# mtlazaro/cg_mrslam

Hardware: AMD Instinct MI355X
Metric: GN iterations/sec on 10k-vertex SE2 graph (final chi2 reported) (higher is better)
Workload: dtype f64; 1 GPU; C2: synthetic 10000-vertex/40000-edge SE2 pose graph per GPU, one step = GraphSLAM::optimize(10) incl. host ordering+symbolic analysis (analysis cache off); graphs=1, parallelism=1 robot sub-graph per GPU x1

## Files before the change

### cg_mrslam_amd/_lib.py

```python
from __future__ import annotations

import ctypes as C
import math
import os
import subprocess

import numpy as np

_HERE = os.path.dirname(os.path.abspath(__file__))
_LIB = None

CGMR_E_CHOLESKY_BASE = -100
CGMR_E_TIMEOUT = -5


class CgmrError(RuntimeError):
    def __init__(self, code, msg):
        super().__init__(f"cgmr error {code}: {msg}")
        self.code = code


def library_path() -> str:
    return os.environ.get("CGMR_LIB") or os.path.join(_HERE, "libcgmr.so")

# ... 746 lines not shown
        return (z, cz, d2) + st

    def observation_covariance(self, poses, fixed, ef, et, meas, info, pair_a, pair_b, obs_kind=None, hyp_meas=None, hyp_info=None,
                               vertex_kind=None, edge_kind=None, kind=None, delta=1.0):
        a, b = self._pair_arrays(pair_a, pair_b)
        n = len(a)
        ok = None if obs_kind is None else np.ascontiguousarray(obs_kind, dtype=np.uint8).reshape(-1)
        if ok is not None and ok.shape != (n,):
            raise ValueError(f"observation kinds: {ok.shape[0]} given for {n} pairs")
        hm = hi = d2 = None
        if hyp_meas is not None:
            hm = np.ascontiguousarray(hyp_meas, dtype=np.float64).reshape(n, 3)
            d2 = np.zeros(n)
        if hyp_info is not None:
            if hm is None:
                raise ValueError("hyp_info needs hyp_meas")
            hi = np.ascontiguousarray(hyp_info, dtype=np.float64).reshape(n, 6)
        z, cz = np.zeros((n, 3)), np.zeros((n, 3, 3))
        st = self._joint_call("cgmr_observation_covariance", poses, fixed, ef, et, meas, info,
                              (C.c_int(n), _ptr(a), _ptr(b), _ptr(ok), _ptr(z), _ptr(cz), _ptr(hm), _ptr(hi), _ptr(d2)), kind, delta,
                              vertex_kind, edge_kind, typed=True)
        return (z, cz, d2) + st

    @staticmethod
    def _adj_bool(words, n):
        if n == 0:
            return np.zeros((0, 0), dtype=bool)
        bits = (words[:, :, None] >> np.arange(64, dtype=np.uint64)) & np.uint64(1)
        return bits.reshape(n, -1)[:, :n].astype(bool)

    @staticmethod
    def _adj_words(adj):
        adj = np.asarray(adj)
        if adj.dtype == np.uint64:
            return np.ascontiguousarray(adj.reshape(adj.shape[0], -1)), adj.shape[0]
        n = adj.shape[0]
        if adj.shape != (n, n):
            raise ValueError(f"adjacency: a square matrix, not {adj.shape}")
        W = (n + 63) // 64
        bits = np.zeros((n, 64 * W), dtype=np.uint64)
        bits[:, :n] = adj.astype(bool)
        words = (bits.reshape(n, W, 64) << np.arange(64, dtype=np.uint64)).sum(axis=2, dtype=np.uint64)
        return np.ascontiguousarray(words), n

    def closure_consistency(self, poses, fixed, ef, et, meas, info, cl_a, cl_b, cl_meas, cl_info, gamma, kind=None, delta=1.0):
        a, b = self._pair_arrays(cl_a, cl_b)
        n = len(a)
        cm = np.ascontiguousarray(cl_meas, dtype=np.float64).reshape(n, 3)
        ci = np.ascontiguousarray(cl_info, dtype=np.float64).reshape(n, 6)
        W = (n + 63) // 64
        d2, words = np.zeros((n, n)), np.zeros((n, W), dtype=np.uint64)
        clique, size, seed = np.full(n, -1, dtype=np.int32), np.zeros(1, dtype=np.int32), np.full(1, -1, dtype=np.int32)
        st = self._joint_call("cgmr_closure_consistency", poses, fixed, ef, et, meas, info,
                              (C.c_int(n), _ptr(a), _ptr(b), _ptr(cm), _ptr(ci), C.c_double(float(gamma)), _ptr(d2), _ptr(words),
                               _ptr(clique), _ptr(size), _ptr(seed)), kind, delta)
        return (d2, self._adj_bool(words, n), clique[:int(size[0])].copy(), int(seed[0])) + st

    def max_clique_greedy(self, adj):
        words, n = self._adj_words(adj)
        clique, size, seed = np.full(n, -1, dtype=np.int32), np.zeros(1, dtype=np.int32), np.full(1, -1, dtype=np.int32)
        self._check(self.lib.cgmr_max_clique_greedy(self.h, C.c_int(n), _ptr(words), _ptr(clique), _ptr(size), _ptr(seed)))
        return clique[:int(size[0])].copy(), int(seed[0])

    def closure_consistency_exact(self, poses, fixed, ef, et, meas, info, cl_a, cl_b, cl_meas, cl_info, gamma,
                                  node_limit=EXACT_DEFAULT_NODE_LIMIT, kind=None, delta=1.0):
        a, b = self._pair_arrays(cl_a, cl_b)
        n = len(a)
        cm = np.ascontiguousarray(cl_meas, dtype=np.float64).reshape(n, 3)
        ci = np.ascontiguousarray(cl_info, dtype=np.float64).reshape(n, 6)
        W = (n + 63) // 64
        d2, words = np.zeros((n, n)), np.zeros((n, W), dtype=np.uint64)
        clique, size, proven = np.full(n, -1, dtype=np.int32), np.zeros(1, dtype=np.int32), np.zeros(1, dtype=np.int32)
        st = self._joint_call("cgmr_closure_consistency_exact", poses, fixed, ef, et, meas, info,
                              (C.c_int(n), _ptr(a), _ptr(b), _ptr(cm), _ptr(ci), C.c_double(float(gamma)), _ptr(d2), _ptr(words),
                               C.c_int64(int(node_limit)), _ptr(clique), _ptr(size), _ptr(proven)), kind, delta)
        return (d2, self._adj_bool(words, n), clique[:int(size[0])].copy(), bool(proven[0])) + st

    def max_clique_exact(self, adj, node_limit=EXACT_DEFAULT_NODE_LIMIT):
        words, n = self._adj_words(adj)
        clique, size, proven = np.full(n, -1, dtype=np.int32), np.zeros(1, dtype=np.int32), np.zeros(1, dtype=np.int32)
        nodes = np.zeros(1, dtype=np.int64)
        self._check(self.lib.cgmr_max_clique_exact(self.h, C.c_int(n), _ptr(words), C.c_int64(int(node_limit)), _ptr(clique),
                                                   _ptr(size), _ptr(proven), _ptr(nodes)))
        return clique[:int(size[0])].copy(), bool(proven[0]), int(nodes[0])

    @staticmethod
    def _inter_arrays(cl_a, peer_pose, peer_cov, cl_meas, cl_info):
        a = np.ascontiguousarray(cl_a, dtype=np.int32).reshape(-1)
        n = len(a)
        pp = np.ascontiguousarray(peer_pose, dtype=np.float64).reshape(n, 3)
        pc = None
        if peer_cov is not None:
            pc = np.ascontiguousarray(peer_cov, dtype=np.float64)
            if pc.shape != (3 * n, 3 * n):
                raise ValueError(f"peer_cov: [{3 * n}, {3 * n}] for {n} candidates, not {pc.shape}")
        cm = np.ascontiguousarray(cl_meas, dtype=np.float64).reshape(n, 3)
        ci = np.ascontiguousarray(cl_info, dtype=np.float64).reshape(n, 6)
        return a, pp, pc, cm, ci

    def closure_consistency_inter(self, poses, fixed, ef, et, meas, info, cl_a, peer_pose, cl_meas, cl_info, gamma, peer_cov=None,
                                  kind=None, delta=1.0):
        a, pp, pc, cm, ci = self._inter_arrays(cl_a, peer_pose, peer_cov, cl_meas, cl_info)
        n = len(a)
        W = (n + 63) // 64
        d2, words = np.zeros((n, n)), np.zeros((n, W), dtype=np.uint64)
        clique, size, seed = np.full(n, -1, dtype=np.int32), np.zeros(1, dtype=np.int32), np.full(1, -1, dtype=np.int32)
        st = self._joint_call("cgmr_closure_consistency_inter", poses, fixed, ef, et, meas, info,
                              (C.c_int(n), _ptr(a), _ptr(pp), _ptr(pc), _ptr(cm), _ptr(ci), C.c_double(float(gamma)), _ptr(d2),
                               _ptr(words), _ptr(clique), _ptr(size), _ptr(seed)), kind, delta)
        return (d2, self._adj_bool(words, n), clique[:int(size[0])].copy(), int(seed[0])) + st

    def closure_consistency_inter_exact(self, poses, fixed, ef, et, meas, info, cl_a, peer_pose, cl_meas, cl_info, gamma,
                                        peer_cov=None, node_limit=EXACT_DEFAULT_NODE_LIMIT, kind=None, delta=1.0):
        a, pp, pc, cm, ci = self._inter_arrays(cl_a, peer_pose, peer_cov, cl_meas, cl_info)
        n = len(a)
        W = (n + 63) // 64
        d2, words = np.zeros((n, n)), np.zeros((n, W), dtype=np.uint64)
        clique, size, proven = np.full(n, -1, dtype=np.int32), np.zeros(1, dtype=np.int32), np.zeros(1, dtype=np.int32)
        st = self._joint_call("cgmr_closure_consistency_inter_exact", poses, fixed, ef, et, meas, info,
                              (C.c_int(n), _ptr(a), _ptr(pp), _ptr(pc), _ptr(cm), _ptr(ci), C.c_double(float(gamma)), _ptr(d2),
                               _ptr(words), C.c_int64(int(node_limit)), _ptr(clique), _ptr(size), _ptr(proven)), kind, delta)
        return (d2, self._adj_bool(words, n), clique[:int(size[0])].copy(), bool(proven[0])) + st

    def set_symbolic_cache(self, on: bool):
        self._check(self.lib.cgmr_set_symbolic_cache(self.h, C.c_int(1 if on else 0)))

    def host_threads_info(self):
        out = np.zeros(5, dtype=np.int32)
        self._check(self.lib.cgmr_host_threads_info(_ptr(out)))
        return {"threads": int(out[0]), "pinned": bool(out[1]), "home_cpu": int(out[2]), "cpus_allowed": int(out[3]),
                "moves": int(out[4])}

    def symbolic_cache_stats(self):
        out = np.zeros(3, dtype=np.int64)
        self._check(self.lib.cgmr_symbolic_cache_stats3(self.h, _ptr(out)))
        return {"hits": int(out[0]), "misses": int(out[1]), "extended": int(out[2])}

    def gn_timeouts(self) -> int:
        self.lib.cgmr_gn_timeouts.restype = C.c_int64
        return int(self.lib.cgmr_gn_timeouts(self.h))

    def switches(self):
        return {r["name"]: r["value"] for r in _switch_rows(self.lib, self.h)}

    def gn_last_timing(self):
        out = np.zeros(5)
        self._check(self.lib.cgmr_gn_last_timing(self.h, _ptr(out)))
        return dict(zip(["order", "structure", "upload", "device", "total"], out.tolist()))

    def set_profiling(self, on: bool):
        self._check(self.lib.cgmr_set_profiling(self.h, C.c_int(1 if on else 0)))

    def gn_kernel_times(self):
        sec = np.zeros(12)
        n = np.zeros(12, dtype=np.int64)
        self._check(self.lib.cgmr_gn_kernel_times_ex(self.h, _ptr(sec), _ptr(n)))
        names = ["linearize", "assemble", "chi2", "front_factor", "front_update", "top_block", "solve_bwd", "update", "front_level"]
        return {k: (float(s), int(c)) for k, s, c in zip(names, sec, n)}

    def pcm_kernel_times(self):
        sec = np.zeros(12)
        n = np.zeros(12, dtype=np.int64)
        self._check(self.lib.cgmr_gn_kernel_times_ex(self.h, _ptr(sec), _ptr(n)))
        return {k: (float(sec[i]), int(n[i])) for i, k in zip((9, 10, 11), ("gram", "consistency", "bits_clique"))}


def _switch_rows(lib, h):
    need = lib.cgmr_switches(h, None, C.c_int(0))
    if need <= 0:
        raise CgmrError(need, "cgmr_switches failed")
    buf = C.create_string_buffer(need)
    lib.cgmr_switches(h, buf, C.c_int(need))
    rows = []
    for line in buf.value.decode().splitlines():
        name, scope, value, effect = line.split("\t")
        rows.append(dict(name=name, scope=scope, value=int(value) if value.lstrip("-").isdigit() else value, effect=effect))
    return rows


def switch_table():
    return _switch_rows(load_library(), None)


_SYM_KEYS = ["free_poses", "offdiag_blocks", "fronts", "levels", "L_doubles", "U_doubles", "max_border",
             "factor_flops", "order_us", "structure_us", "max_children", "max_children_small_border", "panel_doubles",
             "launch_levels", "top_block_fronts", "top_block_cols"]


def gn_symbolic_info_grown(nV0, nE0, nV_steps, nE_steps, ef, et):
    lib = load_library()
    ef = np.ascontiguousarray(ef, dtype=np.int32)
    et = np.ascontiguousarray(et, dtype=np.int32)
    nv = np.ascontiguousarray(nV_steps, dtype=np.int32)
    ne = np.ascontiguousarray(nE_steps, dtype=np.int32)
    out = np.zeros(16, dtype=np.int64)
    nV = int(nv[-1]) if len(nv) else nV0
    perm = np.zeros(nV, dtype=np.int32)
    next_ = C.c_int32(0)
    rc = lib.cgmr_gn_symbolic_info_grown(C.c_int(nV0), C.c_int(nE0), C.c_int(len(nv)), _ptr(nv), _ptr(ne), _ptr(ef), _ptr(et),
                                         _ptr(out), _ptr(perm), C.byref(next_))
    if rc != 0:
        raise CgmrError(rc, "cgmr_gn_symbolic_info_grown rejected the graph")
    return dict(zip(_SYM_KEYS, out.tolist())), perm, int(next_.value)


def gn_front_table(nV, fixed, ef, et):
    lib = load_library()
    fixed = np.ascontiguousarray(fixed, dtype=np.uint8)
    ef = np.ascontiguousarray(ef, dtype=np.int32)
    et = np.ascontiguousarray(et, dtype=np.int32)
    cap = max(64, int(nV))
    out = np.zeros(6 * cap, dtype=np.int32)
    n = lib.cgmr_debug_fronts(C.c_int(nV), _ptr(fixed), C.c_int(len(ef)), _ptr(ef), _ptr(et), C.c_int(cap), _ptr(out))
    if n < 0 or n > cap:
        raise CgmrError(n, "cgmr_debug_fronts rejected the graph")
    return out[:6 * n].reshape(n, 6)


def gn_symbolic_info(nV, fixed, ef, et, want_perm=False):
    lib = load_library()
    fixed = np.ascontiguousarray(fixed, dtype=np.uint8)
    ef = np.ascontiguousarray(ef, dtype=np.int32)
    et = np.ascontiguousarray(et, dtype=np.int32)
    out = np.zeros(16, dtype=np.int64)
    perm = np.zeros(nV, dtype=np.int32) if want_perm else None
    rc = lib.cgmr_gn_symbolic_info(C.c_int(nV), _ptr(fixed), C.c_int(len(ef)), _ptr(ef), _ptr(et), _ptr(out),
                                   _ptr(perm))
    if rc != 0:
        raise CgmrError(rc, "cgmr_gn_symbolic_info rejected the graph")
    keys = ["free_poses", "offdiag_blocks", "fronts", "levels", "L_doubles", "U_doubles", "max_border",
            "factor_flops", "order_us", "structure_us", "max_children", "max_children_small_border", "panel_doubles",
            "launch_levels", "top_block_fronts", "top_block_cols"]
    info = dict(zip(keys, out.tolist()))
    return (info, perm) if want_perm else info
```

### cg_mrslam_amd/csrc/cgmr_api.cpp

```cpp
#include "factor_model.h"
#include "host_call.h"

#include <algorithm>
#include <cstdio>
#include <cmath>
#include <cstring>
#include <vector>

namespace cgmr {

int robust_setup(cgmr_ctx* ctx, const cgmr_robust* rk, int nE, bool dev, GnEdges& Ed, const char* who) {
  if (!rk) return 0;
  const size_t n = (size_t)std::max(nE, 0);
  std::vector<uint8_t> hk;
  std::vector<double> hd;
  const uint8_t* ck = rk->kind;
  const double* cd = rk->delta;
  if (dev && n > 0 && (rk->kind || rk->delta)) {
    if (rk->kind) { hk.resize(n); HIP_TRY(ctx, hipMemcpyAsync(hk.data(), rk->kind, n, hipMemcpyDeviceToHost, ctx->stream)); ck = hk.data(); }
    if (rk->delta) { hd.resize(n); HIP_TRY(ctx, hipMemcpyAsync(hd.data(), rk->delta, 8 * n, hipMemcpyDeviceToHost, ctx->stream)); cd = hd.data(); }
    HIP_TRY(ctx, hipStreamSynchronize(ctx->stream));
  }
  bool ok = rk->default_kind >= CGMR_RK_NONE && rk->default_kind <= CGMR_RK_DCS;
  if (ok && !rk->kind && !rk->delta) ok = robust_valid(rk->default_kind, rk->default_delta);
// ... 688 lines not shown
                         const int32_t* et, const double* meas, const double* info, int nP, const int32_t* pair_a,
                         const int32_t* pair_b, double* cov_aa_out, double* cov_ab_out, double* cov_bb_out, const cgmr_robust* rk) {
  return joint_driver(ctx, "cgmr_marginals_pairs", 1, host_call(nV, poses, fixed, nE, ef, et, meas, info, {false, rk}), nP, pair_a, pair_b, cov_aa_out, cov_ab_out,
      cov_bb_out, nullptr, nullptr);
}

int cgmr_relative_covariance(cgmr_ctx* ctx, int nV, const double* poses, const uint8_t* fixed, int nE, const int32_t* ef,
                             const int32_t* et, const double* meas, const double* info, int nP, const int32_t* pair_a,
                             const int32_t* pair_b, double* rel_xyt_out, double* rel_cov_out, const double* hyp_meas,
                             const double* hyp_info, double* d2_out, const cgmr_robust* rk) {
  return joint_driver(ctx, "cgmr_relative_covariance", 2, host_call(nV, poses, fixed, nE, ef, et, meas, info, {false, rk}), nP, pair_a, pair_b, rel_xyt_out,
      rel_cov_out, d2_out, hyp_meas, hyp_info);
}

int cgmr_marginals_joint_typed(cgmr_ctx* ctx, int nV, const double* poses, const uint8_t* fixed, int nE, const int32_t* ef,
                               const int32_t* et, const double* meas, const double* info, int nK, const int32_t* query,
                               double* cov_out, const cgmr_factor_types* types, const cgmr_robust* rk) {
  return joint_driver(ctx, "cgmr_marginals_joint_typed", 0, host_call(nV, poses, fixed, nE, ef, et, meas, info, {false, rk, types}), nK, query, nullptr, cov_out,
      nullptr, nullptr, nullptr, nullptr);
}
int cgmr_marginals_pairs_typed(cgmr_ctx* ctx, int nV, const double* poses, const uint8_t* fixed, int nE, const int32_t* ef,
                               const int32_t* et, const double* meas, const double* info, int nP, const int32_t* pair_a,
                               const int32_t* pair_b, double* cov_aa_out, double* cov_ab_out, double* cov_bb_out,
                               const cgmr_factor_types* types, const cgmr_robust* rk) {
  return joint_driver(ctx, "cgmr_marginals_pairs_typed", 1, host_call(nV, poses, fixed, nE, ef, et, meas, info, {false, rk, types}), nP, pair_a, pair_b, cov_aa_out,
      cov_ab_out, cov_bb_out, nullptr, nullptr);
}

int cgmr_observation_covariance(cgmr_ctx* ctx, int nV, const double* poses, const uint8_t* fixed, int nE, const int32_t* ef,
                                const int32_t* et, const double* meas, const double* info, int nP, const int32_t* pair_a,
                                const int32_t* pair_b, const uint8_t* obs_kind, double* z_out, double* cov_out,
                                const double* hyp_meas, const double* hyp_info, double* d2_out, const cgmr_factor_types* types,
                                const cgmr_robust* rk) {
  return joint_driver(ctx, "cgmr_observation_covariance", 2, host_call(nV, poses, fixed, nE, ef, et, meas, info, {false, rk, types}), nP, pair_a, pair_b, z_out,
      cov_out, d2_out, hyp_meas, hyp_info, true, obs_kind);
}

int cgmr_closure_consistency(cgmr_ctx* ctx, int nV, const double* poses, const uint8_t* fixed, int nE, const int32_t* ef,
                             const int32_t* et, const double* meas, const double* info, int nC, const int32_t* cl_a,
                             const int32_t* cl_b, const double* cl_meas, const double* cl_info, double gamma, double* d2_out,
                             uint64_t* adj_out, int32_t* clique_out, int32_t* clique_size_out, int32_t* seed_out,
                             const cgmr_robust* rk) {
  return pcm_driver(ctx, host_call(nV, poses, fixed, nE, ef, et, meas, info, {false, rk}), nC, cl_a, cl_b, cl_meas, cl_info, gamma, d2_out, adj_out, clique_out,
      clique_size_out, seed_out);
}

int cgmr_max_clique_greedy(cgmr_ctx* ctx, int n, const uint64_t* adj_bits, int32_t* clique_out, int32_t* clique_size_out,
                           int32_t* seed_out) {
  if (!ctx) return CGMR_E_INVALID;
  return clique_driver(ctx, n, adj_bits, clique_out, clique_size_out, seed_out);
}

int cgmr_closure_consistency_exact(cgmr_ctx* ctx, int nV, const double* poses, const uint8_t* fixed, int nE, const int32_t* ef,
                                   const int32_t* et, const double* meas, const double* info, int nC, const int32_t* cl_a,
                                   const int32_t* cl_b, const double* cl_meas, const double* cl_info, double gamma, double* d2_out,
                                   uint64_t* adj_out, int64_t node_limit, int32_t* clique_out, int32_t* clique_size_out,
                                   int32_t* proven_out, const cgmr_robust* rk) {
  const CliqueExact ex{node_limit, proven_out, nullptr};
  return pcm_driver(ctx, host_call(nV, poses, fixed, nE, ef, et, meas, info, {false, rk}), nC, cl_a, cl_b, cl_meas, cl_info, gamma, d2_out, adj_out, clique_out,
      clique_size_out, nullptr, &ex);
}

int cgmr_closure_consistency_inter(cgmr_ctx* ctx, int nV, const double* poses, const uint8_t* fixed, int nE, const int32_t* ef,
                                   const int32_t* et, const double* meas, const double* info, int nC, const int32_t* cl_a,
                                   const double* peer_pose, const double* peer_cov, const double* cl_meas, const double* cl_info,
                                   double gamma, double* d2_out, uint64_t* adj_out, int32_t* clique_out, int32_t* clique_size_out,
                                   int32_t* seed_out, const cgmr_robust* rk) {
  const PcmInter inter{peer_pose, peer_cov};
  return pcm_driver(ctx, host_call(nV, poses, fixed, nE, ef, et, meas, info, {false, rk}), nC, cl_a, nullptr, cl_meas, cl_info, gamma, d2_out, adj_out,
      clique_out, clique_size_out, seed_out, nullptr, &inter);
}

int cgmr_closure_consistency_inter_exact(cgmr_ctx* ctx, int nV, const double* poses, const uint8_t* fixed, int nE, const int32_t* ef,
                                         const int32_t* et, const double* meas, const double* info, int nC, const int32_t* cl_a,
                                         const double* peer_pose, const double* peer_cov, const double* cl_meas,
                                         const double* cl_info, double gamma, double* d2_out, uint64_t* adj_out, int64_t node_limit,
                                         int32_t* clique_out, int32_t* clique_size_out, int32_t* proven_out, const cgmr_robust* rk) {
  const CliqueExact ex{node_limit, proven_out, nullptr};
  const PcmInter inter{peer_pose, peer_cov};
  return pcm_driver(ctx, host_call(nV, poses, fixed, nE, ef, et, meas, info, {false, rk}), nC, cl_a, nullptr, cl_meas, cl_info, gamma, d2_out, adj_out,
      clique_out, clique_size_out, nullptr, &ex, &inter);
}

int cgmr_max_clique_exact(cgmr_ctx* ctx, int n, const uint64_t* adj_bits, int64_t node_limit, int32_t* clique_out,
                          int32_t* clique_size_out, int32_t* proven_out, int64_t* nodes_out) {
  if (!ctx) return CGMR_E_INVALID;
  const CliqueExact ex{node_limit, proven_out, nodes_out};
  return clique_driver(ctx, n, adj_bits, clique_out, clique_size_out, nullptr, &ex);
}

int cgmr_set_symbolic_cache(cgmr_ctx* ctx, int on) {
  if (!ctx) return CGMR_E_INVALID;
  ctx->sym_cache_on = on != 0;
  ctx->sym_valid = false;
  return CGMR_OK;
}

int cgmr_host_threads_info(int32_t out[5]) {
  if (!out) return CGMR_E_INVALID;
  int v[5];
  host_pool_info(v);
  for (int k = 0; k < 5; k++) out[k] = v[k];
  return CGMR_OK;
}

int cgmr_symbolic_cache_stats(const cgmr_ctx* ctx, int64_t out[2]) {
  if (!ctx || !out) return CGMR_E_INVALID;
  out[0] = ctx->sym_hits; out[1] = ctx->sym_misses + ctx->sym_extended;
  return CGMR_OK;
}

int cgmr_symbolic_cache_stats3(const cgmr_ctx* ctx, int64_t out[3]) {
  if (!ctx || !out) return CGMR_E_INVALID;
  out[0] = ctx->sym_hits; out[1] = ctx->sym_misses; out[2] = ctx->sym_extended;
  return CGMR_OK;
}

int64_t cgmr_gn_timeouts(const cgmr_ctx* ctx) { return ctx ? ctx->gn_timeouts : -1; }

int cgmr_switches(const cgmr_ctx* ctx, char* buf, int cap) {
  if (cap < 0 || (cap > 0 && !buf)) return CGMR_E_INVALID;
  const Switches defaults;
  return list_switches(ctx ? ctx->sw : defaults, ctx ? process_switches() : defaults, buf, cap);
}

int cgmr_gn_last_timing(const cgmr_ctx* ctx, double out[5]) {
  if (!ctx || !out) return CGMR_E_INVALID;
  memcpy(out, ctx->timing, sizeof(double) * 5);
  return CGMR_OK;
}

int cgmr_set_profiling(cgmr_ctx* ctx, int on) {
  if (!ctx) return CGMR_E_INVALID;
  ctx->profiling = on != 0;
  memset(ctx->ksec, 0, sizeof ctx->ksec);
  memset(ctx->klaunch, 0, sizeof ctx->klaunch);
  ctx->ev_cls.clear();
  if (on && ctx->ev_pool.empty()) {
    HIP_TRY(ctx, hipSetDevice(ctx->device));
    ctx->ev_pool.resize(2 * 2048);
    for (hipEvent_t& e : ctx->ev_pool)
      if (hipEventCreate(&e) != hipSuccess) { ctx->ev_pool.clear(); return set_err(ctx, CGMR_E_HIP, "hipEventCreate failed"); }
  }
  return CGMR_OK;
}

int cgmr_gn_kernel_times(const cgmr_ctx* ctx, double seconds_out[8], int64_t launches_out[8]) {
  if (!ctx || !seconds_out || !launches_out) return CGMR_E_INVALID;
  memcpy(seconds_out, ctx->ksec, sizeof(double) * 8);
  memcpy(launches_out, ctx->klaunch, sizeof(int64_t) * 8);
  return CGMR_OK;
}

extern "C" int cgmr_gn_kernel_times_ex(const cgmr_ctx* ctx, double seconds_out[12], int64_t launches_out[12]) {
  if (!ctx || !seconds_out || !launches_out) return CGMR_E_INVALID;
  memcpy(seconds_out, ctx->ksec, sizeof(double) * 12);
  memcpy(launches_out, ctx->klaunch, sizeof(int64_t) * 12);
  return CGMR_OK;
}

}
```

### cg_mrslam_amd/csrc/cgmr_ctx.h

```cpp
#pragma once
#include <hip/hip_runtime_api.h>

#include <cstdint>
#include <string>
#include <utility>
#include <vector>

#include "../../include/cgmr.h"
#include "gn_device.h"
#include "gn_symbolic.h"
#include "switches.h"

namespace cgmr {
struct Arena {
  char* ptr = nullptr;
  size_t cap = 0;
};
}

struct cgmr_ctx {
  cgmr::Switches sw;
  int device = 0;
  int n_cus = 0;
  hipStream_t stream = nullptr;
  bool own_stream = false;
  std::string err;
  std::vector<std::pair<void*, const void*>> graveyard;
  cgmr::Arena gn_arena;
  cgmr::Arena io_arena;
  cgmr::Arena mt_arena;
  cgmr::Arena mtab_arena;
  bool mtab_valid = false;
  double mtab_key[6] = {0, 0, 0, 0, 0, 0};
  cgmr::Arena rep_arena;
  cgmr::Arena mg_arena;
  cgmr::Arena si_arena;
  cgmr::Arena lm_arena;
  cgmr::Arena rk_arena;
  cgmr::Arena ty_arena;
  cgmr::Arena mix_arena;
  int64_t lm_stats[2] = {0, 0};
  cgmr::Arena dl_arena;
  int64_t dl_stats[3] = {0, 0, 0};
  cgmr::Arena gnc_arena;
  int64_t gnc_stats[2] = {0, 0};
  cgmr::Arena st_arena;
  char* pinned_st = nullptr;
  size_t pinned_st_cap = 0;
  hipEvent_t ev_st_copied = nullptr;
  struct StView { int32_t *vperm = nullptr, *ef = nullptr, *et = nullptr, *off_row = nullptr, *off_col = nullptr, *offbase = nullptr, *asm_ptr = nullptr, *asm_src = nullptr; bool fresh = false; } st_view;
  hipStream_t side = nullptr;
  hipEvent_t side_fork = nullptr, side_tail = nullptr;
  bool side_busy = false;
  bool side_used = false;
  char* pinned = nullptr;
  size_t pinned_cap = 0;
  char* pinned_mask = nullptr;
  size_t pinned_mask_cap = 0;
  bool sym_cache_on = true;
  bool sym_valid = false;
  int sym_nV = 0;
  int sym_chi_cap = 0;
  std::vector<int32_t> sym_ef, sym_et;
  int64_t gn_timeouts = 0;
  bool fwd_merge_any = true;
  int64_t sym_hits = 0, sym_misses = 0, sym_extended = 0;
  std::vector<uint8_t> vmask;
  cgmr::Symbolic sym;
  cgmr::GnDevice gn;
  double* poses_out_host = nullptr;
  double timing[5] = {0, 0, 0, 0, 0};
  long long trace_n = 0;
  double trace_sum[4] = {0, 0, 0, 0};
  double match_seconds = 0;
  int64_t match_pairs = 0, match_slow_pairs = 0;
  int64_t match_ext_pairs = 0;
  int64_t match_redo_why[3] = {0, 0, 0};
  int64_t match_shape[4] = {0, 0, 0, 0};
  int64_t match_redo_pairs = 0;
  bool profiling = false;
  double ksec[12] = {0};
  int64_t klaunch[12] = {0};
  std::vector<hipEvent_t> ev_pool;
  std::vector<int> ev_cls;
  hipEvent_t ev0 = nullptr, ev1 = nullptr, ev_a = nullptr, ev_b = nullptr;
};

namespace cgmr {
double wall_s();
int set_err(cgmr_ctx* ctx, int code, const char* fmt, ...);
int arena_reserve(cgmr_ctx* ctx, Arena& A, size_t bytes);
int pinned_reserve(cgmr_ctx* ctx, size_t bytes);
int side_stream(cgmr_ctx* ctx);
int side_fork(cgmr_ctx* ctx);
int side_mark(cgmr_ctx* ctx);
int side_join_host(cgmr_ctx* ctx);
int side_join_stream(cgmr_ctx* ctx, hipStream_t st);
}
```

### cg_mrslam_amd/csrc/gn_device.h

```cpp
#pragma once
#include <hip/hip_runtime_api.h>

#include <cstdint>
#include <vector>

#include "gn_symbolic.h"

namespace cgmr {

struct GncState;
struct Switches;

struct GnDevice {
  const Switches* sw = nullptr;
  int nV = 0, nE = 0, nf = 0, nb = 0, nlevels = 0, nfronts = 0;
  FrontDesc* fronts = nullptr;
  FrontDesc* fronts_lv = nullptr;
  int32_t *rows = nullptr, *children = nullptr, *rel = nullptr, *inv = nullptr;
  WorkRec* work = nullptr;
  int32_t *level_fronts = nullptr, *tiles = nullptr, *blk_dst = nullptr, *b_dst = nullptr, *asm_ptr = nullptr, *asm_src = nullptr, *vperm = nullptr;
  int32_t *ef = nullptr, *et = nullptr;
  int32_t *off_row = nullptr, *off_col = nullptr;
  uint8_t* cmask = nullptr;
  double *term = nullptr, *Ablk = nullptr, *bvec = nullptr, *yvec = nullptr, *xvec = nullptr, *uvec = nullptr;
  double *Lbuf = nullptr, *Ubuf = nullptr;
  double* Pan = nullptr;
  int64_t pan_doubles = 0;
  bool pan_clean = false;
  double* chi2 = nullptr;
  int* status = nullptr;
  int* ready = nullptr;
  int bwd_chain_level = 0;
  int bwd_chain_wgs = 4;
  int njobs = 1;
  long long job_stride = 0, pose_stride = 0;
  int top_nfronts = 0, top_c0 = 0, top_ncols = 0, top_nchild = 0, top_nblk = 0;
  int32_t *top_fronts = nullptr, *top_children = nullptr, *top_blocks = nullptr;
  int nlevels_full = 0;
  std::vector<int32_t> h_flevel_ptr;
  std::vector<int32_t> h_level_ptr, h_tile_ptr, h_work_ptr;
  std::vector<uint8_t> h_level_leaf;
  std::vector<int32_t> h_level_chunk;
  std::vector<uint8_t> h_level_mergeable;
  std::vector<uint8_t> h_level_merge;
  std::vector<int32_t> h_level_chrows;
};

struct RobustArgs {
  const uint8_t* kind = nullptr;
  const double* delta = nullptr;
  double* stats = nullptr;
  double delta0 = 1.0;
  int kind0 = 0;
};
struct TypedArgs {
  const uint8_t* edge_kind = nullptr;
};
struct GncArgs {
  double* weight = nullptr;
  const double* barc_sq = nullptr;
  const uint8_t* known = nullptr;
  const GncState* S = nullptr;
  double* r_out = nullptr;
  int mode = 0;
};
struct MixArgs {
  const int32_t* cptr = nullptr;
  const double* cmeas = nullptr;
  const double* cinfo = nullptr;
  const double* coff = nullptr;
  int32_t* sel_out = nullptr;
};
struct UnaryLists {
  int n = 0;
  const int32_t *vertex = nullptr, *ptr = nullptr, *edge = nullptr;
};

struct GnEdges {
  const double *meas_a = nullptr, *info_a = nullptr, *meas_b = nullptr, *info_b = nullptr;
  int nA = 0, n_active = 0;
  bool robust = false, typed = false, gnc = false, gnc_own_only = false, mix = false;
  RobustArgs rk;
  TypedArgs ty;
  UnaryLists unary;
  GncArgs ga;
  MixArgs mx;
  int chordal_stage = 0;
};
struct AsmBuild {
  int nE = 0, nf = 0, nb = 0;
  const int32_t *vperm = nullptr, *ef = nullptr, *et = nullptr, *off_row = nullptr, *offbase = nullptr;
  int32_t *asm_ptr = nullptr, *asm_src = nullptr, *ekey = nullptr, *cnt = nullptr, *longlist = nullptr, *tmp = nullptr;
};
void launch_build_asm(hipStream_t st, const AsmBuild& B);
void launch_build_maps(hipStream_t st, const GnDevice& D, const int32_t* offbase, const int32_t* rec0);
void launch_linearize(hipStream_t st, const GnDevice& D, const double* poses, const GnEdges& Ed, int chi_only);
void launch_chi2(hipStream_t st, const GnDevice& D, double* out);
void launch_assemble(hipStream_t st, const GnDevice& D);
void launch_add_unary(hipStream_t st, const GnDevice& D, const GnEdges& Ed);
void gn_init_kernels();
void launch_factor_level(hipStream_t st, const GnDevice& D, int level, bool write_l11c);
void launch_update_level(hipStream_t st, const GnDevice& D, int level);
void launch_front_level(hipStream_t st, const GnDevice& D, int level, bool write_l11c);
void choose_fwd_merge(GnDevice& D, int slots_div, bool off, bool any_size = false);
void launch_bwd_level(hipStream_t st, const GnDevice& D, int level);
void launch_bwd_chain(hipStream_t st, const GnDevice& D);
int bwd_chain_capacity(int per_cu);
void choose_bwd_chain(GnDevice& D, int slots_div, bool levelwise);
void launch_update(hipStream_t st, const GnDevice& D, double* poses);
void launch_top_block(hipStream_t st, const GnDevice& D, bool store_l, bool write_l11c, bool clear_panels, bool make_z);
void launch_invert_fronts(hipStream_t st, const GnDevice& D, bool top_too = false);
struct CondJobDev { int32_t nq, gauge, gauge_id, out_slot; };
struct MargBatch {
  const CondJobDev* jobs = nullptr;
  long long marg_stride = 0, est_stride = 0, info_stride = 0, wire_stride = 0;
};
void launch_marginals(hipStream_t st, const GnDevice& D, int nK, const int32_t* d_qcol, int m, double* Y, double* Uv,
                      double* part, double* G, double* cov, int chunk, int nchunk, uint8_t* live, const MargBatch* batch = nullptr,
                      bool y_is_zero = false);
void launch_label(hipStream_t st, int nK, const int32_t* d_qvert, int gauge, const double* poses, const double* cov,
                  double* est, double* info, int* flags, const GnDevice* D = nullptr, const MargBatch* batch = nullptr);
void launch_marginals_solve(hipStream_t st, const GnDevice& D, int nK, const int32_t* d_qcol, int m, double* Y, double* Uv,
                            uint8_t* live, const MargBatch* batch = nullptr, bool y_is_zero = false);
struct JointGram {
  const int32_t* tiles = nullptr;
  long long ntile = 0;
  int rows = 0, nsplit = 1;
  double *part = nullptr, *G = nullptr;
};
void joint_gram_split(int n, long long nwg, int* rows_out, int* nsplit_out);
void launch_joint_gram(hipStream_t st, int n, int m, const double* Y, const JointGram& J);
void launch_joint_extract(hipStream_t st, int nK, const int32_t* slot, const double* G, double* cov);
void launch_pairs_extract(hipStream_t st, int nP, const int32_t* pr, const double* G, double* aa, double* ab, double* bb);
void launch_relative_cov(hipStream_t st, int nP, const int32_t* pa, const int32_t* pb, const double* poses, const double* aa,
                         const double* ab, const double* bb, const double* hyp_meas, const double* hyp_info, double* rel,
                         double* rel_cov, double* d2);
void launch_observation_cov(hipStream_t st, int nP, const int32_t* pa, const int32_t* pb, const uint8_t* kind, const double* poses,
                            const double* aa, const double* ab, const double* bb, const double* hyp_meas, const double* hyp_info,
                            double* z, double* cov, double* d2);
constexpr int kSelinvTileRows = 64;
struct SelinvPlan {
  double* Sig = nullptr;
  const int64_t* soff = nullptr;
  const int32_t* tiles = nullptr;
  std::vector<int32_t> h_tile_ptr;
};
void launch_selinv(hipStream_t st, const GnDevice& D, const SelinvPlan& P, int nV, int nE, const int32_t* vcol,
                   const int32_t* col_front, double* cov, double* cross);

}
```

### cg_mrslam_amd/csrc/gn_host.cpp

```cpp
#include "gn_host.h"
#include "init_device.h"

#include <algorithm>
#include <chrono>
#include <cstdarg>
#include <cstring>

namespace cgmr {

double wall_s() {
  using namespace std::chrono;
  return duration_cast<duration<double>>(steady_clock::now().time_since_epoch()).count();
}

int set_err(cgmr_ctx* ctx, int code, const char* fmt, ...) {
  char buf[512];
  va_list ap;
  va_start(ap, fmt);
  vsnprintf(buf, sizeof buf, fmt, ap);
  va_end(ap);
  if (ctx) ctx->err = buf;
  return code;
}

int side_stream(cgmr_ctx* ctx) {
  if (ctx->side) return 0;
  HIP_TRY(ctx, hipStreamCreateWithFlags(&ctx->side, hipStreamNonBlocking));
  HIP_TRY(ctx, hipEventCreateWithFlags(&ctx->side_fork, hipEventDisableTiming));
  HIP_TRY(ctx, hipEventCreateWithFlags(&ctx->side_tail, hipEventDisableTiming));
  return 0;
}

int side_fork(cgmr_ctx* ctx) {
  int rc = side_stream(ctx);
  if (rc) return rc;
  HIP_TRY(ctx, hipEventRecord(ctx->side_fork, ctx->stream));
  HIP_TRY(ctx, hipStreamWaitEvent(ctx->side, ctx->side_fork, 0));
  return 0;
}

int side_mark(cgmr_ctx* ctx) {
  HIP_TRY(ctx, hipEventRecord(ctx->side_tail, ctx->side));
  ctx->side_busy = true;
  return 0;
}

int side_join_host(cgmr_ctx* ctx) {
  if (!ctx->side_busy) return 0;
  HIP_TRY(ctx, hipEventSynchronize(ctx->side_tail));
  ctx->side_busy = false;
  return 0;
}

int side_join_stream(cgmr_ctx* ctx, hipStream_t st) {
  if (!ctx->side_busy) return 0;
  HIP_TRY(ctx, hipStreamWaitEvent(st, ctx->side_tail, 0));
  return 0;
}

int arena_reserve(cgmr_ctx* ctx, Arena& A, size_t bytes) {
  if (bytes <= A.cap) return 0;
  if (A.ptr) { ctx->graveyard.push_back({A.ptr, nullptr}); A.ptr = nullptr; }
  size_t want = std::max(bytes + bytes / 2, 2 * A.cap) + (1 << 20);
  A.cap = 0;
  hipError_t e = hipMalloc((void**)&A.ptr, want);
  if (e != hipSuccess) return set_err(ctx, CGMR_E_ALLOC, "hipMalloc(%zu): %s", want, hipGetErrorString(e));
  A.cap = want;
  return 0;
}

int pinned_reserve(cgmr_ctx* ctx, size_t bytes) {
  if (bytes <= ctx->pinned_cap) return 0;
  if (ctx->pinned) { (void)hipStreamSynchronize(ctx->stream); (void)side_join_host(ctx); (void)hipHostFree(ctx->pinned); ctx->pinned = nullptr; ctx->pinned_cap = 0; }
  size_t want = std::max(2 * bytes, (size_t)4 << 20);
  hipError_t e = hipHostMalloc((void**)&ctx->pinned, want, hipHostMallocDefault);
  if (e != hipSuccess) return set_err(ctx, CGMR_E_ALLOC, "hipHostMalloc(%zu): %s", want, hipGetErrorString(e));
  ctx->pinned_cap = want;
  return 0;
}

int pinned_mask_reserve(cgmr_ctx* ctx, size_t bytes) {
  if (bytes <= ctx->pinned_mask_cap) return 0;
  if (ctx->pinned_mask) { (void)hipStreamSynchronize(ctx->stream); (void)side_join_host(ctx); (void)hipHostFree(ctx->pinned_mask); ctx->pinned_mask = nullptr; ctx->pinned_mask_cap = 0; }
  size_t want = bytes + bytes / 2 + 4096;
  hipError_t e = hipHostMalloc((void**)&ctx->pinned_mask, want, hipHostMallocDefault);
  if (e != hipSuccess) return set_err(ctx, CGMR_E_ALLOC, "hipHostMalloc(%zu): %s", want, hipGetErrorString(e));
  ctx->pinned_mask_cap = want;
  return 0;
}

int gn_upload_early(cgmr_ctx* ctx, const Symbolic& S, const int32_t* ef, const int32_t* et, const int32_t* offbase) {
  const size_t nV = (size_t)S.nV, nE = (size_t)S.nE, nb = (size_t)S.nb, nf = (size_t)S.nf, nkeys = nf + nb;
  BlobLayout B;
  const size_t o_vperm = B.add<int32_t>(nV), o_ef = B.add<int32_t>(nE), o_et = B.add<int32_t>(nE), o_orow = B.add<int32_t>(nb),
               o_ocol = B.add<int32_t>(nb), o_obase = B.add<int32_t>(nf + 1);
  const size_t up_bytes = (B.off + 255) & ~size_t(255);
  B.off = up_bytes;
  const size_t o_asmp = B.add<int32_t>(nkeys + 1), o_asms = B.add<int32_t>(3 * nE + 4), o_cnt = B.add<int32_t>(nkeys + 4),
               o_ekey = B.add<int32_t>(nE), o_long = B.add<int32_t>(3 * nE / 16 + 2), o_tmp = B.add<int32_t>(3 * nE + 4);
  int rc = side_join_stream(ctx, ctx->stream);
  if (rc) return rc;
  rc = arena_reserve(ctx, ctx->st_arena, B.off + 256);
  if (rc) return rc;
  if (!ctx->ev_st_copied) HIP_TRY(ctx, hipEventCreateWithFlags(&ctx->ev_st_copied, hipEventDisableTiming));
  else HIP_TRY(ctx, hipEventSynchronize(ctx->ev_st_copied));
  if (up_bytes > ctx->pinned_st_cap) {
    if (ctx->pinned_st) { (void)hipHostFree(ctx->pinned_st); ctx->pinned_st = nullptr; ctx->pinned_st_cap = 0; }
    const size_t want = std::max(2 * up_bytes, (size_t)2 << 20);
    hipError_t e = hipHostMalloc((void**)&ctx->pinned_st, want, hipHostMallocDefault);
    if (e != hipSuccess) return set_err(ctx, CGMR_E_ALLOC, "hipHostMalloc(%zu): %s", want, hipGetErrorString(e));
    ctx->pinned_st_cap = want;
  }
  char* h = ctx->pinned_st;
  host_run_tasks(4, [&](int task) {
    switch (task) {
      case 0: memcpy(h + o_ef, ef, 4 * nE); break;
      case 1: memcpy(h + o_et, et, 4 * nE); break;
      case 2: memcpy(h + o_orow, S.off_row.data(), 4 * nb); memcpy(h + o_obase, offbase, 4 * (nf + 1)); break;
      default: memcpy(h + o_ocol, S.off_col.data(), 4 * nb); memcpy(h + o_vperm, S.vperm.data(), 4 * nV); break;
    }
  });
  char* d = ctx->st_arena.ptr;
  HIP_TRY(ctx, hipMemcpyAsync(d, h, up_bytes, hipMemcpyHostToDevice, ctx->stream));
  HIP_TRY(ctx, hipEventRecord(ctx->ev_st_copied, ctx->stream));
  cgmr_ctx::StView& V = ctx->st_view;
  V.vperm = (int32_t*)(d + o_vperm); V.ef = (int32_t*)(d + o_ef); V.et = (int32_t*)(d + o_et);
  V.off_row = (int32_t*)(d + o_orow); V.off_col = (int32_t*)(d + o_ocol); V.offbase = (int32_t*)(d + o_obase);
  V.asm_ptr = (int32_t*)(d + o_asmp); V.asm_src = (int32_t*)(d + o_asms);
  V.fresh = true;
  AsmBuild A;
  A.nE = S.nE; A.nf = S.nf; A.nb = S.nb;
  A.vperm = V.vperm; A.ef = V.ef; A.et = V.et; A.off_row = V.off_row; A.offbase = (const int32_t*)(d + o_obase);
  A.asm_ptr = V.asm_ptr; A.asm_src = V.asm_src; A.ekey = (int32_t*)(d + o_ekey); A.cnt = (int32_t*)(d + o_cnt);
  A.longlist = (int32_t*)(d + o_long); A.tmp = (int32_t*)(d + o_tmp);
  launch_build_asm(ctx->stream, A);
  HIP_TRY(ctx, hipGetLastError());
  return 0;
}

int gn_upload(cgmr_ctx* ctx, const Symbolic& S, int iters) {
  cgmr_ctx::StView& V = ctx->st_view;
  if (S.nf == 0) V = cgmr_ctx::StView();
  else if (!V.fresh) return set_err(ctx, CGMR_E_INVALID, "structure upload of an analysis without its device pass (AnalyzeHooks::blocks_ready)");
  V.fresh = false;
  if (3 * (int64_t)S.max_ns + kFrontW > 32767)
    return set_err(ctx, CGMR_E_INVALID, "a front has %d border poses; at most %d are supported", S.max_ns, (32767 - kFrontW) / 3);
  GnDevice& D = ctx->gn;
  D.nV = S.nV; D.nE = S.nE; D.nf = S.nf; D.nb = S.nb;
  D.nfronts = (int)S.fronts.size();
  D.nlevels = (int)S.gn_level_ptr.size() - 1;
  D.h_level_ptr = S.gn_level_ptr;
  D.nlevels_full = (int)S.level_ptr.size() - 1;
  D.h_flevel_ptr = S.level_ptr;
  const std::vector<int32_t>& LF = S.gn_level_fronts;
  const Switches& sw = ctx->sw;
  D.h_tile_ptr.assign(D.nlevels + 1, 0);
  D.h_work_ptr.assign(D.nlevels + 1, 0);
  D.h_level_chrows.assign(D.nlevels, 1);
  D.h_level_leaf.assign(D.nlevels, 1);
  D.h_level_chunk.assign(D.nlevels, kChunkRows);
  D.h_level_mergeable.assign(D.nlevels, 1);
  std::vector<std::vector<int32_t>> sched(D.nlevels);
  for (int q = 0; q < (int)LF.size(); q++) {
    const FrontDesc& F = S.fronts[LF[q]];
    if (F.ns > 0) sched[std::min(F.sched_t, D.nlevels - 1)].push_back(LF[q]);
  }
  for (auto& v : sched) std::sort(v.begin(), v.end());
  std::vector<int32_t> rec0_of(2 * S.fronts.size(), 0);
  for (size_t f = 0; f < S.fronts.size(); f++) rec0_of[2 * f] = -1;
  for (int l = 0; l < D.nlevels; l++) {
    for (int q = S.gn_level_ptr[l]; q < S.gn_level_ptr[l + 1]; q++)
      if (S.fronts[LF[q]].nchild > 0) D.h_level_leaf[l] = 0;
    int chunk_rows = D.h_level_leaf[l] ? sw.leaf_chunk : sw.mid_chunk;
    if (!D.h_level_leaf[l] && S.gn_level_ptr[l + 1] - S.gn_level_ptr[l] <= sw.top_chunk_fronts) chunk_rows = std::min(chunk_rows, sw.top_chunk);
    D.h_level_chunk[l] = chunk_rows;
    int nwork = 0;
    for (int q = S.gn_level_ptr[l]; q < S.gn_level_ptr[l + 1]; q++) {
      const int r = 3 * S.fronts[LF[q]].ns;
      const int nchunk = std::max(1, (r + chunk_rows - 1) / chunk_rows);
      rec0_of[2 * LF[q]] = D.h_work_ptr[l] + nwork;
      rec0_of[2 * LF[q] + 1] = nchunk;
      nwork += nchunk;
      D.h_level_chrows[l] = std::max(D.h_level_chrows[l], std::min(r, chunk_rows) + 1);
    }
    int xload[8] = {0, 0, 0, 0, 0, 0, 0, 0};
    for (int f : sched[l]) {
      if (S.fronts[f].nchild > kWorkChildren) D.h_level_mergeable[l] = 0;
      const int T = (3 * S.fronts[f].ns + 31) / 32;
      *std::min_element(xload, xload + 8) += T * (T + 1) / 2;
    }
    D.h_tile_ptr[l + 1] = D.h_tile_ptr[l] + 8 * *std::max_element(xload, xload + 8);
    D.h_work_ptr[l + 1] = D.h_work_ptr[l] + nwork;
  }
  const size_t n_tiles = (size_t)D.h_tile_ptr[D.nlevels], n_work = (size_t)D.h_work_ptr[D.nlevels];
  BlobLayout B;
  size_t o_fronts = B.add<FrontDesc>(S.fronts.size());
  size_t o_fronts_lv = B.add<FrontDesc>(S.fronts.size());
  size_t o_rows = B.add<int32_t>(S.rows.size());
  size_t o_children = B.add<int32_t>(S.children.size());
  size_t o_lf = B.add<int32_t>(S.level_fronts.size());
  size_t o_tiles = B.add<int32_t>(3 * n_tiles);
  size_t o_rec0 = B.add<int32_t>(rec0_of.size());
  size_t o_tf = B.add<int32_t>(S.top_fronts.size()), o_tc = B.add<int32_t>(S.top_children.size()), o_tb = B.add<int32_t>(S.top_blocks.size());
  size_t blob_bytes = (B.off + 255) & ~size_t(255);
  BlobLayout N;
  N.off = blob_bytes;
  size_t o_term = N.add<double>((size_t)34 * S.nE);
  size_t o_A = N.add<double>((size_t)9 * (S.nf + S.nb));
  size_t o_b = N.add<double>((size_t)3 * S.nf);
  size_t o_y = N.add<double>((size_t)3 * S.nf);
  size_t o_x = N.add<double>((size_t)3 * S.nf);
  size_t o_u = N.add<double>((size_t)3 * S.rows.size() + 3);
  size_t o_L = N.add<double>((size_t)S.L_doubles + 1);
  size_t o_U = N.add<double>((size_t)S.U_doubles + 1);
  size_t o_pan = N.add<double>((size_t)S.pan_doubles + 2);
  size_t o_chi = N.add<double>((size_t)iters + 2);
  size_t o_status = N.add<int>(4);
  size_t o_ready = N.add<int>(S.fronts.size() + 4);
  size_t o_cmask = N.add<uint8_t>((size_t)S.nf + 16);
  size_t o_rel = N.add<int32_t>((size_t)S.n_rel + 4), o_inv = N.add<int32_t>((size_t)S.n_inv + 4);
  size_t o_bdst = N.add<int32_t>((size_t)S.nf + S.nb + 4), o_rdst = N.add<int32_t>((size_t)S.nf + 4);
  size_t o_work = N.add<WorkRec>(n_work + 1);
  size_t total = N.off + 256;
  int rc = arena_reserve(ctx, ctx->gn_arena, total);
  if (rc) return rc;
  rc = pinned_reserve(ctx, blob_bytes);
  if (rc) return rc;
  char* h = ctx->pinned;
  auto put = [&](size_t off, const void* src, size_t bytes) { if (bytes) memcpy(h + off, src, bytes); };
  host_run_tasks(6, [&](int task) {
    switch (task) {
      case 0: {
        int32_t* tiles = reinterpret_cast<int32_t*>(h + o_tiles);
        for (int l = 0; l < D.nlevels; l++) {
          int32_t* tl = tiles + 3 * (size_t)D.h_tile_ptr[l];
          const int slots = D.h_tile_ptr[l + 1] - D.h_tile_ptr[l];
          for (int k = 0; k < slots; k++) { tl[3 * k] = -1; tl[3 * k + 1] = 0; tl[3 * k + 2] = 0; }
          int xload[8] = {0, 0, 0, 0, 0, 0, 0, 0};
          for (int f : sched[l]) {
            const int T = (3 * S.fronts[f].ns + 31) / 32;
            const int x = (int)(std::min_element(xload, xload + 8) - xload);
            for (int ti = 0; ti < T; ti++)
              for (int tj = 0; tj <= ti; tj++) {
                int32_t* e = tl + 3 * (size_t)(8 * xload[x]++ + x);
                e[0] = rec0_of[2 * f]; e[1] = ti; e[2] = tj;
              }
          }
        }
        break;
      }
      case 1:
        put(o_rec0, rec0_of.data(), rec0_of.size() * 4);
        put(o_children, S.children.data(), S.children.size() * 4);
        break;
      case 2:
        put(o_fronts, S.fronts.data(), S.fronts.size() * sizeof(FrontDesc));
        break;
      case 3: {
        FrontDesc* lv = reinterpret_cast<FrontDesc*>(h + o_fronts_lv);
        for (size_t q = 0; q < S.fronts.size(); q++) {
          if (q < LF.size()) lv[q] = S.fronts[LF[q]];
          else memset(&lv[q], 0, sizeof(FrontDesc));
        }
        break;
      }
      case 4:
        put(o_lf, S.level_fronts.data(), S.level_fronts.size() * 4);
        put(o_tf, S.top_fronts.data(), S.top_fronts.size() * 4);
        put(o_tc, S.top_children.data(), S.top_children.size() * 4);
        put(o_tb, S.top_blocks.data(), S.top_blocks.size() * 4);
        break;
      default:
        put(o_rows, S.rows.data(), S.rows.size() * 4);
        break;
    }
  });
  char* d = ctx->gn_arena.ptr;
  rc = side_join_stream(ctx, ctx->stream);
  if (rc) return rc;
  HIP_TRY(ctx, hipMemcpyAsync(d, h, blob_bytes, hipMemcpyHostToDevice, ctx->stream));
  D.fronts = (FrontDesc*)(d + o_fronts);
  D.fronts_lv = (FrontDesc*)(d + o_fronts_lv);
  D.rows = (int32_t*)(d + o_rows);
  D.children = (int32_t*)(d + o_children);
  D.rel = (int32_t*)(d + o_rel);
  D.inv = (int32_t*)(d + o_inv);
  D.blk_dst = (int32_t*)(d + o_bdst);
  D.b_dst = (int32_t*)(d + o_rdst);
  D.level_fronts = (int32_t*)(d + o_lf);
  D.tiles = (int32_t*)(d + o_tiles);
  D.work = (WorkRec*)(d + o_work);
  D.asm_ptr = V.asm_ptr; D.asm_src = V.asm_src; D.vperm = V.vperm; D.ef = V.ef; D.et = V.et; D.off_row = V.off_row; D.off_col = V.off_col;
  D.cmask = (uint8_t*)(d + o_cmask);
  D.top_fronts = (int32_t*)(d + o_tf); D.top_children = (int32_t*)(d + o_tc); D.top_blocks = (int32_t*)(d + o_tb);
  D.top_nfronts = (int)S.top_fronts.size(); D.top_c0 = S.top_c0; D.top_ncols = 3 * S.top_nposes;
  D.top_nchild = (int)S.top_children.size(); D.top_nblk = (int)S.top_blocks.size() / 3;
  D.term = (double*)(d + o_term);
  D.Ablk = (double*)(d + o_A);
  D.bvec = (double*)(d + o_b);
  D.yvec = (double*)(d + o_y);
  D.xvec = (double*)(d + o_x);
  D.uvec = (double*)(d + o_u);
  D.Lbuf = (double*)(d + o_L);
  D.Ubuf = (double*)(d + o_U);
  launch_build_maps(ctx->stream, D, V.offbase, (const int32_t*)(d + o_rec0));
  HIP_TRY(ctx, hipGetLastError());
  D.Pan = (double*)(d + o_pan);
  D.pan_clean = false;
  D.pan_doubles = S.pan_doubles;
  D.chi2 = (double*)(d + o_chi);
  D.status = (int*)(d + o_status);
  D.ready = (int*)(d + o_ready);
  choose_bwd_chain(D, ctx->side_used ? 2 : 1, false);
  choose_fwd_merge(D, ctx->side_used ? 2 : 1, false, ctx->fwd_merge_any);
  return 0;
}

int gn_replicas(cgmr_ctx* ctx, int n, GnDevice& D, size_t* stride_out) {
  const Symbolic& S = ctx->sym;
  BlobLayout N;
  size_t o_term = N.add<double>((size_t)34 * S.nE), o_A = N.add<double>((size_t)9 * (S.nf + S.nb)), o_b = N.add<double>((size_t)3 * S.nf),
         o_y = N.add<double>((size_t)3 * S.nf), o_x = N.add<double>((size_t)3 * S.nf), o_u = N.add<double>((size_t)3 * S.rows.size() + 3),
         o_L = N.add<double>((size_t)S.L_doubles + 1), o_U = N.add<double>((size_t)S.U_doubles + 1),
         o_pan = N.add<double>((size_t)S.pan_doubles + 2), o_chi = N.add<double>(8),
         o_status = N.add<int>(4), o_ready = N.add<int>(S.fronts.size() + 4), o_cmask = N.add<uint8_t>((size_t)S.nf + 16);
  const size_t per = (N.off + 255) & ~size_t(255);
  int rc = arena_reserve(ctx, ctx->rep_arena, per * (size_t)std::max(n, 1) + 256);
  if (rc) return rc;
  *stride_out = per;
  char* d = ctx->rep_arena.ptr;
  D = ctx->gn;
  D.term = (double*)(d + o_term); D.Ablk = (double*)(d + o_A); D.bvec = (double*)(d + o_b); D.yvec = (double*)(d + o_y);
  D.xvec = (double*)(d + o_x); D.uvec = (double*)(d + o_u); D.Lbuf = (double*)(d + o_L); D.Ubuf = (double*)(d + o_U); D.Pan = (double*)(d + o_pan); D.pan_clean = false;
  D.chi2 = (double*)(d + o_chi); D.status = (int*)(d + o_status); D.ready = (int*)(d + o_ready); D.cmask = (uint8_t*)(d + o_cmask);
  return 0;
}

int analyze_next(Symbolic& sym, const Switches& sw, bool have_prev, int prev_nV, const std::vector<int32_t>& pef, const std::vector<int32_t>& pet,
                 const GnSystem& N, const AnalyzeHooks* hooks) {
  int n_common = 0;
  if (have_prev && N.nV >= prev_nV && !pef.empty()) {
    const int lim = std::min(N.nE, (int)pef.size());
    while (n_common < lim && pef[n_common] == N.ef[n_common] && pet[n_common] == N.et[n_common]) n_common++;
  }
  const int old_nE = (int)pef.size();
  const bool grown = n_common > 0 && (n_common == old_nE || (N.n_hub_vertices > 0 && 2 * n_common >= old_nE));
  if (grown) {
    Symbolic old = std::move(sym);
    return analyze(N.nV, nullptr, N.nE, N.ef, N.et, sym, sw, &old, n_common == old_nE && N.nE >= old_nE ? -1 : n_common, N.hub_vertices, N.n_hub_vertices, hooks);
  }
  return analyze(N.nV, nullptr, N.nE, N.ef, N.et, sym, sw, nullptr, -1, N.hub_vertices, N.n_hub_vertices, hooks);
}

int prepare_structure(cgmr_ctx* ctx, int nV, int nE, const int32_t* ef, const int32_t* et, int iters, const int32_t* hub_vertices,
                      int n_hub_vertices) {
  const bool hit = ctx->sym_cache_on && ctx->sym_valid && ctx->sym_nV == nV && (int)ctx->sym_ef.size() == nE &&
                   iters <= ctx->sym_chi_cap &&
                   (nE == 0 || (memcmp(ctx->sym_ef.data(), ef, sizeof(int32_t) * nE) == 0 &&
                                memcmp(ctx->sym_et.data(), et, sizeof(int32_t) * nE) == 0));
  if (hit) {
    ctx->sym_hits++;
    ctx->sym.t_order = ctx->sym.t_struct = ctx->sym.t_upload = 0;
    return 0;
  }
  const bool have_prev = ctx->sym_cache_on && ctx->sym_valid;
  ctx->sym_valid = false;
  AnalyzeHooks hooks;
  int hook_rc = 0;
  hooks.blocks_ready = [&](const Symbolic& S, const int32_t* offbase) { hook_rc = gn_upload_early(ctx, S, ef, et, offbase); return hook_rc ? -100 : 0; };
  int rc = analyze_next(ctx->sym, ctx->sw, have_prev, ctx->sym_nV, ctx->sym_ef, ctx->sym_et, {nV, nullptr, nullptr, nE, ef, et, hub_vertices, n_hub_vertices}, &hooks);
  if (rc == -100) return hook_rc;
  if (rc == 0 && ctx->sym.extended) ctx->sym_extended++; else ctx->sym_misses++;
  if (rc) return set_err(ctx, CGMR_E_INVALID, "graph structure rejected (edge index out of range)");
  const int chi_cap = std::max(iters, 30);
  const double tu0 = wall_s();
  rc = gn_upload(ctx, ctx->sym, chi_cap);
  if (rc) return rc;
  ctx->sym.t_upload = wall_s() - tu0;
  if (ctx->sym_cache_on) {
    ctx->sym_nV = nV;
    ctx->sym_ef.assign(ef, ef + nE);
    ctx->sym_et.assign(et, et + nE);
    ctx->sym_valid = true;
  }
  ctx->sym_chi_cap = chi_cap;
  return 0;
}

int prepare_pass(cgmr_ctx* ctx, const uint8_t* fixed, int nE, const int32_t* ef, const int32_t* et, int n_active) {
  const Symbolic& S = ctx->sym;
  GnDevice& D = ctx->gn;
  hipStream_t st = ctx->stream;
  ctx->vmask.assign(S.nV, 0);
  if (fixed) for (int v = 0; v < S.nV; v++) ctx->vmask[v] = fixed[v] ? 1 : 0;
  if (n_active < nE) {
    std::vector<uint8_t> live(S.nV, 0);
    for (int k = 0; k < n_active; k++) { live[ef[k]] = 1; live[et[k]] = 1; }
    for (int v = 0; v < S.nV; v++) if (!live[v]) ctx->vmask[v] = 1;
  }
  HIP_TRY(ctx, hipMemsetAsync(D.status, 0, 16, st));
  if (S.nf == 0) return 0;
  int rc = pinned_mask_reserve(ctx, (size_t)S.nf);
  if (rc) return rc;
  char* pm = ctx->pinned_mask;
  for (int c = 0; c < S.nf; c++) pm[c] = (char)ctx->vmask[S.perm[c]];
  HIP_TRY(ctx, hipMemcpyAsync(D.cmask, pm, (size_t)S.nf, hipMemcpyHostToDevice, st));
  return 0;
}

void profile_collect(cgmr_ctx* ctx) {
  for (size_t k = 0; k < ctx->ev_cls.size(); k++) {
    float ms = 0;
    if (hipEventElapsedTime(&ms, ctx->ev_pool[2 * k], ctx->ev_pool[2 * k + 1]) == hipSuccess) ctx->ksec[ctx->ev_cls[k]] += 1e-3 * ms;
  }
  ctx->ev_cls.clear();
}

void gn_pass(cgmr_ctx* ctx, double* d_poses, const GnEdges& Ed, const GnPassOpts& o) {
  gn_pass_on(ctx, ctx->gn, ctx->stream, d_poses, Ed, o);
}

void gn_pass_on(cgmr_ctx* ctx, GnDevice& D, hipStream_t st, double* d_poses, const GnEdges& Ed, const GnPassOpts& o) {
  const bool write_l11c = o.write_l11c;
  KTimer T{ctx, st};
  T.run(0, 1, [&] { launch_linearize(st, D, d_poses, Ed, o.chi_only ? 1 : 0); });
  if (o.chi_only || D.nf == 0) {
    T.run(2, 1, [&] { launch_chi2(st, D, D.chi2 + o.chi_slot); });
    return;
  }
  if (D.pan_doubles > 0 && !D.pan_clean) {
    if (D.njobs > 1) (void)hipMemset2DAsync(D.Pan, (size_t)D.job_stride, 0, sizeof(double) * (size_t)D.pan_doubles, (size_t)D.njobs, st);
    else (void)hipMemsetAsync(D.Pan, 0, sizeof(double) * (size_t)D.pan_doubles, st);
  }
  D.pan_clean = false;
  T.run(1, 1, [&] { launch_assemble(st, D); });
  if (Ed.typed && Ed.unary.n > 0) T.run(1, 1, [&] { launch_add_unary(st, D, Ed); });
  if (o.after_assemble) o.after_assemble(st, D, o.after_assemble_arg);
  const bool trace = ctx->sw.trace_launches;
  if (trace)
    fprintf(stderr, "[cgmr] arena %p .. %p; work %p rel %p Pan %p Ablk %p bvec %p yvec %p uvec %p Lbuf %p Ubuf %p chi2 %p\n",
            (void*)ctx->gn_arena.ptr, (void*)(ctx->gn_arena.ptr + ctx->gn_arena.cap), (void*)D.work, (void*)D.rel, (void*)D.Pan,
            (void*)D.Ablk, (void*)D.bvec, (void*)D.yvec, (void*)D.uvec, (void*)D.Lbuf, (void*)D.Ubuf, (void*)D.chi2);
  for (int l = 0; l < D.nlevels; l++) {
    if (trace) {
      int maxr = 0, maxc = 0;
      for (int q = D.h_level_ptr[l]; q < D.h_level_ptr[l + 1]; q++) {
        const FrontDesc& F = ctx->sym.fronts[ctx->sym.gn_level_fronts[q]];
        maxr = std::max(maxr, 3 * F.ns);
        for (int k = 0; k < F.nchild; k++) maxc = std::max(maxc, 3 * ctx->sym.fronts[ctx->sym.children[F.child_off + k]].ns);
      }
      if (D.h_level_ptr[l + 1] - D.h_level_ptr[l] <= 2)
        for (int q = D.h_level_ptr[l]; q < D.h_level_ptr[l + 1]; q++) {
          const FrontDesc& F = ctx->sym.fronts[ctx->sym.gn_level_fronts[q]];
          fprintf(stderr, "[cgmr]   front nc %d ns %d na %d nchild %d a_cnt %d L_off %lld U_off %lld:", F.nc, F.ns, F.na, F.nchild, F.a_cnt, (long long)F.L_off, (long long)F.U_off);
          for (int k = 0; k < F.nchild; k++) { const FrontDesc& G = ctx->sym.fronts[ctx->sym.children[F.child_off + k]]; fprintf(stderr, " child(ns %d na %d U_off %lld)", G.ns, G.na, (long long)G.U_off); }
          fprintf(stderr, "\n");
        }
      fprintf(stderr, "[cgmr] level %d: %d fronts, %d work items, max r %d, max child rows %d\n", l,
              D.h_level_ptr[l + 1] - D.h_level_ptr[l], D.h_work_ptr[l + 1] - D.h_work_ptr[l], maxr, maxc);
    }
    if (l < (int)D.h_level_merge.size() && D.h_level_merge[l]) { T.run(8, 1, [&] { launch_front_level(st, D, l, write_l11c); }); continue; }
    T.run(3, 1, [&] { launch_factor_level(st, D, l, write_l11c); });
    if (D.h_tile_ptr[l + 1] > D.h_tile_ptr[l]) T.run(4, 1, [&] { launch_update_level(st, D, l); });
  }
  const bool clear_in_top = ctx->sw.clear_in_top;
  const bool chain = o.solve && D.bwd_chain_level < D.nlevels;
  if (D.top_nfronts > 0) {
    T.run(5, 1, [&] { launch_top_block(st, D, write_l11c, write_l11c, clear_in_top, chain); });
    D.pan_clean = clear_in_top && D.pan_doubles > 0;
  } else if (chain) {
    T.run(5, 1, [&] { launch_invert_fronts(st, D); });
  }
  if (!o.solve) return;
  if (D.bwd_chain_level < D.nlevels) T.run(6, 1, [&] { launch_bwd_chain(st, D); });
  for (int l = D.bwd_chain_level - 1; l >= 0; l--) T.run(6, 1, [&] { launch_bwd_level(st, D, l); });
  if (o.update_poses)
    T.run(7, 1, [&] { if (Ed.chordal_stage == kChordalRotation) launch_apply_rotation(st, D, d_poses); else launch_update(st, D, d_poses); });
}

int LevelwiseScope::arm(hipStream_t st, int it0) {
  count_timeout(ctx);
  armed = true;
  chain_was = D.bwd_chain_level;
  merge_was = D.h_level_merge;
  D.bwd_chain_level = D.nlevels;
  D.h_level_merge.assign(D.nlevels, 0);
  const int fresh[4] = {0, it0, 0, 0};
  HIP_TRY(ctx, hipMemcpyAsync(D.status, fresh, sizeof fresh, hipMemcpyHostToDevice, st));
  return 0;
}

int gn_run(cgmr_ctx* ctx, const GnSystem& S, const GnEdges& Ed, int iters, double* chi2_out) {
  GnCall call(ctx, S);
  int rc = call.prepare(Ed.n_active, iters);
  if (rc) return rc;
  GnDevice& D = ctx->gn;
  hipStream_t st = ctx->stream;
  GnEdges Ei = Ed;
  Ei.rk.stats = nullptr;
  Ei.mx.sel_out = nullptr;
  auto queue_from = [&](int it0) {
    GnPassOpts o;
    for (o.chi_slot = it0; o.chi_slot < iters; o.chi_slot++) gn_pass(ctx, S.d_poses, Ei, o);
    o.chi_only = true;
    gn_pass(ctx, S.d_poses, Ed, o);
  };
  rc = call.begin();
  if (rc) return rc;
  const bool graph_mode = ctx->sw.graph, trace_launches = ctx->sw.trace_launches;
  hipGraph_t graph = nullptr;
  hipGraphExec_t graph_exec = nullptr;
  if (graph_mode && !ctx->profiling && !trace_launches && iters >= 2 && st != nullptr && D.nf > 0 && !Ed.mix) {
    gn_init_kernels();
    HIP_TRY(ctx, hipStreamBeginCapture(st, hipStreamCaptureModeThreadLocal));
    gn_pass(ctx, S.d_poses, Ei, GnPassOpts());
    HIP_TRY(ctx, hipStreamEndCapture(st, &graph));
    HIP_TRY(ctx, hipGraphInstantiate(&graph_exec, graph, nullptr, nullptr, 0));
    for (int it = 0; it < iters; it++) HIP_TRY(ctx, hipGraphLaunch(graph_exec, st));
    queue_from(iters);
  } else {
    queue_from(0);
  }
  HIP_TRY(ctx, hipEventRecord(ctx->ev1, st));
  const double t3 = wall_s();
  std::vector<double> chi(iters + 1);
  int status4[4] = {0, 0, 0, 0};
  const std::initializer_list<GnCall::Readback> results = {{chi.data(), D.chi2, sizeof(double) * (iters + 1)}, {status4, D.status, sizeof status4}};
  rc = call.wait(results);
  if (rc) return rc;
  {
    if (ctx->sw.gn_trace) {
      const double t4 = wall_s();
      ctx->trace_n++; ctx->trace_sum[0] += call.t1 - call.t0; ctx->trace_sum[1] += call.t2 - call.t1; ctx->trace_sum[2] += t3 - call.t2; ctx->trace_sum[3] += t4 - t3;
    }
  }
  if (graph_exec) (void)hipGraphExecDestroy(graph_exec);
  if (graph) (void)hipGraphDestroy(graph);
  if (status4[2] != 0 && status4[0] > 0) {
    const int it0 = status4[0] - 1;
    LevelwiseScope levelwise(ctx, D);
    rc = levelwise.arm(st, it0);
    if (rc) return rc;
    queue_from(it0);
    rc = call.wait(results);
    if (rc) return rc;
    if (status4[2] != 0) return set_err(ctx, CGMR_E_TIMEOUT, "backward solve: a bounded device-side wait ran out twice");
  }
  const int status = status4[0];
  call.finish();
  if (chi2_out) memcpy(chi2_out, chi.data(), sizeof(double) * (iters + 1));
  if (status != 0)
    return set_err(ctx, CGMR_E_CHOLESKY_BASE - (status - 1),
                   "Cholesky failed (non-positive pivot) in GN iteration %d; poses left at the last good update",
                   status - 1);
  return CGMR_OK;
}

void initial_guess_host(int nV, double* poses, const uint8_t* fixed, int nE, const int32_t* ef, const int32_t* et,
                        const double* meas) {
  auto norm = [](double t) {
    const double pi = 3.14159265358979323846;
    if (t >= -pi && t < pi) return t;
    return t - 2 * pi * std::floor((t + pi) / (2 * pi));
  };
  std::vector<int> deg(nV + 1, 0);
  for (int k = 0; k < nE; k++) { deg[ef[k] + 1]++; deg[et[k] + 1]++; }
  for (int v = 0; v < nV; v++) deg[v + 1] += deg[v];
  std::vector<int> inc(2 * (size_t)nE + 1), pos(deg.begin(), deg.end() - 1);
  for (int k = 0; k < nE; k++) { inc[pos[ef[k]]++] = k; inc[pos[et[k]]++] = k; }
  std::vector<uint8_t> seen(nV, 0);
  std::vector<int> queue;
  queue.reserve(nV);
  for (int v = 0; v < nV; v++) if (fixed[v] && deg[v + 1] > deg[v]) { seen[v] = 1; queue.push_back(v); }
  for (size_t qh = 0; qh < queue.size(); qh++) {
    int u = queue[qh];
    for (int p = deg[u]; p < deg[u + 1]; p++) {
      int k = inc[p];
      int w = (ef[k] == u) ? et[k] : ef[k];
      if (seen[w]) continue;
      seen[w] = 1;
      const double* a = poses + 3 * (size_t)u;
      double z[3] = {meas[3 * k], meas[3 * k + 1], meas[3 * k + 2]};
      if (ef[k] != u) {
        double c = std::cos(z[2]), s = std::sin(z[2]);
        double ix = -(c * z[0] + s * z[1]), iy = -(-s * z[0] + c * z[1]);
        z[0] = ix; z[1] = iy; z[2] = -z[2];
      }
      double c = std::cos(a[2]), s = std::sin(a[2]);
      double* o = poses + 3 * (size_t)w;
      o[0] = a[0] + c * z[0] - s * z[1];
      o[1] = a[1] + s * z[0] + c * z[1];
      o[2] = norm(a[2] + z[2]);
      queue.push_back(w);
    }
  }
}

void symbolic_info_out(const Symbolic& S, int nV, int64_t out[16], int32_t* perm_out) {
  out[0] = S.nf; out[1] = S.nb; out[2] = (int64_t)S.fronts.size(); out[3] = (int64_t)S.level_ptr.size() - 1;
  out[4] = S.L_doubles; out[5] = S.U_doubles; out[6] = S.max_ns; out[7] = (int64_t)S.flops;
  out[8] = (int64_t)(1e6 * S.t_order); out[9] = (int64_t)(1e6 * S.t_struct);
  out[10] = out[11] = out[12] = 0;
  out[13] = (int64_t)S.gn_level_ptr.size() - 1; out[14] = (int64_t)S.top_fronts.size(); out[15] = 3 * (int64_t)S.top_nposes;
  for (const FrontDesc& F : S.fronts) {
    out[12] += pan_size(F.ns) * F.pan_slots;
    out[10] = std::max<int64_t>(out[10], F.nchild);
    if (F.ns >= 1 && F.ns <= 32) out[11] = std::max<int64_t>(out[11], F.nchild);
  }
  if (perm_out) memcpy(perm_out, S.vperm.data(), sizeof(int32_t) * nV);
}

}
```

### cg_mrslam_amd/csrc/gn_host.h

```cpp
#pragma once
#include <cmath>
#include <cstdio>
#include <initializer_list>

#include "cgmr_ctx.h"

#define HIP_TRY(ctx, call)                                                                      \
  do {                                                                                          \
    hipError_t e_ = (call);                                                                     \
    if (e_ != hipSuccess) return set_err(ctx, CGMR_E_HIP, "%s: %s", #call, hipGetErrorString(e_)); \
  } while (0)

namespace cgmr {

inline bool robust_valid(int kind, double delta) {
  return kind == CGMR_RK_NONE || (kind > CGMR_RK_NONE && kind <= CGMR_RK_DCS && std::isfinite(delta) && delta > 0);
}

int pinned_mask_reserve(cgmr_ctx* ctx, size_t bytes);
int prepare_structure(cgmr_ctx* ctx, int nV, int nE, const int32_t* ef, const int32_t* et, int iters,
                      const int32_t* hub_vertices = nullptr, int n_hub_vertices = 0);
int prepare_pass(cgmr_ctx* ctx, const uint8_t* fixed, int nE, const int32_t* ef, const int32_t* et, int n_active);
int gn_replicas(cgmr_ctx* ctx, int n, GnDevice& D, size_t* stride_out);
struct Layout256 {
  size_t off = 0;
  explicit Layout256(size_t base = 0) : off(base) {}
  size_t add(size_t bytes) { off = (off + 255) & ~size_t(255); const size_t o = off; off += bytes; return o; }
};
struct MargLayout {
  static constexpr int chunk = 2048;
  int m = 0, n = 0, nchunk = 0;
  size_t o_qc = 0, o_qv = 0, o_Y = 0, o_U = 0, o_part = 0, o_G = 0, o_cov = 0, o_est = 0, o_info = 0, o_fl = 0, o_live = 0, end = 0;
  MargLayout() = default;
  MargLayout(int nq, int nf, size_t rows, int nfronts, size_t base = 0, bool flags_first = false)
      : m(((4 * nq + 15) / 16) * 16),
        n(3 * nf), nchunk((n + chunk - 1) / chunk) {
    Layout256 L(base);
    o_qc = L.add(4 * (size_t)nq); o_qv = L.add(4 * (size_t)nq); o_Y = L.add(8 * (size_t)n * m);
    o_U = L.add(8 * (3 * rows + 3) * m); o_part = L.add(8 * (size_t)nchunk * 16 * m); o_G = L.add(8 * (size_t)16 * m);
    o_cov = L.add(72 * (size_t)nq);
    if (flags_first) o_fl = L.add(4 * (size_t)nq);
    o_est = L.add(24 * (size_t)nq); o_info = L.add(48 * (size_t)nq);
    if (!flags_first) o_fl = L.add(4 * (size_t)nq);
    o_live = L.add((size_t)(nfronts > 1 ? nfronts : 1) * (m / 16));
    end = L.off;
  }
};
struct GnPassOpts {
  int chi_slot = 0;
  bool chi_only = false;
  bool solve = true;
  bool update_poses = true;
  bool write_l11c = false;
  void (*after_assemble)(hipStream_t st, const GnDevice& D, void* arg) = nullptr;
  void* after_assemble_arg = nullptr;
};
void gn_pass_on(cgmr_ctx* ctx, GnDevice& D, hipStream_t st, double* d_poses, const GnEdges& Ed, const GnPassOpts& o);
void gn_pass(cgmr_ctx* ctx, double* d_poses, const GnEdges& Ed, const GnPassOpts& o);
inline void count_timeout(cgmr_ctx* ctx) {
  ctx->gn_timeouts++;
  ctx->fwd_merge_any = false;
}
struct LevelwiseScope {
  cgmr_ctx* ctx;
  GnDevice& D;
  bool armed = false;
  int chain_was = 0;
  std::vector<uint8_t> merge_was;
  LevelwiseScope(cgmr_ctx* c, GnDevice& d) : ctx(c), D(d) {}
  LevelwiseScope(const LevelwiseScope&) = delete;
  LevelwiseScope& operator=(const LevelwiseScope&) = delete;
  int arm(hipStream_t st, int it0 = 0);
  ~LevelwiseScope() {
    if (!armed) return;
    D.bwd_chain_level = chain_was;
    D.h_level_merge.swap(merge_was);
  }
};
struct GnSystem {
  int nV; double* d_poses; const uint8_t* fixed; int nE; const int32_t *ef, *et;
  const int32_t* hub_vertices = nullptr; int n_hub_vertices = 0;
};
inline int prepare_structure(cgmr_ctx* ctx, const GnSystem& S, int iters) {
  return prepare_structure(ctx, S.nV, S.nE, S.ef, S.et, iters, S.hub_vertices, S.n_hub_vertices);
}
struct LmOut { double *chi2, *lambda; int32_t *trials, *iters_done; };
struct DlOut { double *chi2, *delta; int32_t *trials, *step, *iters_done; };
struct GncOut { double *mu, *cost; int32_t *partial, *outer_done; double *weight, *edge_chi2; };
int gn_run(cgmr_ctx* ctx, const GnSystem& S, const GnEdges& Ed, int iters, double* chi2_out);
int chordal_run(cgmr_ctx* ctx, const GnSystem& S, const GnEdges& Ed, int stages, const uint8_t* in_rot, const uint8_t* in_tr,
                double* chi2_out, int32_t* counts_out);
int lm_run(cgmr_ctx* ctx, const GnSystem& S, const GnEdges& Ed, int iters, const cgmr_lm_params* params, const LmOut& out);
int dl_run(cgmr_ctx* ctx, const GnSystem& S, const GnEdges& Ed, int iters, const cgmr_dl_params* params, const DlOut& out);
bool dl_params_ok(const cgmr_dl_params* params);
int gnc_run(cgmr_ctx* ctx, const GnSystem& S, const GnEdges& Ed, const cgmr_gnc_params& P, const double* barc_sq,
            const uint8_t* known, const GncOut& out);
bool gnc_params_ok(const cgmr_gnc_params* params);
cgmr_gnc_params gnc_params_default();
double gnc_default_barc_sq(int dim);
void initial_guess_host(int nV, double* poses, const uint8_t* fixed, int nE, const int32_t* ef, const int32_t* et,
                        const double* meas);
int analyze_next(Symbolic& sym, const Switches& sw, bool have_prev, int prev_nV, const std::vector<int32_t>& pef, const std::vector<int32_t>& pet,
                 const GnSystem& N, const AnalyzeHooks* hooks = nullptr);
void symbolic_info_out(const Symbolic& S, int nV, int64_t out[16], int32_t* perm_out);
void host_pool_info(int out[5]);
void profile_collect(cgmr_ctx* ctx);

struct BlobLayout {
  size_t off = 0;
  template <typename T>
  size_t add(size_t count) {
    off = (off + 15) & ~size_t(15);
    size_t o = off;
    off += count * sizeof(T);
    return o;
  }
};

struct KTimer {
  cgmr_ctx* ctx;
  hipStream_t st;
  template <typename Fn>
  void run(int cls, int nlaunch, Fn&& fn) {
    if (ctx->sw.trace_launches) {
      fprintf(stderr, "[cgmr] launch class %d (0 lin 1 asm 2 chi2 3 factor 4 update 5 top 6 bwd 7 poses 8 factor+update)\n", cls);
      fn();
      hipError_t e = hipStreamSynchronize(st);
      fprintf(stderr, "[cgmr]   done: %s\n", hipGetErrorString(e));
      return;
    }
    if (!ctx->profiling || st != ctx->stream || 2 * (ctx->ev_cls.size() + 1) > ctx->ev_pool.size()) { fn(); return; }
    const size_t k = ctx->ev_cls.size();
    (void)hipEventRecord(ctx->ev_pool[2 * k], ctx->stream);
    fn();
    (void)hipEventRecord(ctx->ev_pool[2 * k + 1], ctx->stream);
    ctx->ev_cls.push_back(cls);
    ctx->klaunch[cls] += nlaunch;
  }
};

struct GnCall {
  cgmr_ctx* ctx;
  const GnSystem& sys;
  double t0, t1 = 0, t2 = 0;
  double* poses_host = nullptr;
  struct Readback { void* dst; const void* src; size_t bytes; };

  GnCall(cgmr_ctx* c, const GnSystem& s) : ctx(c), sys(s), t0(wall_s()) {}
  int prepare(int n_active, int chi_slots) {
    int rc = prepare_structure(ctx, sys, chi_slots);
    if (rc) return rc;
    t1 = wall_s();
    rc = prepare_pass(ctx, sys.fixed, sys.nE, sys.ef, sys.et, n_active);
    t2 = wall_s();
    return rc;
  }
  int begin() {
    HIP_TRY(ctx, hipEventRecord(ctx->ev0, ctx->stream));
    poses_host = ctx->poses_out_host;
    ctx->poses_out_host = nullptr;
    return 0;
  }
  int wait(std::initializer_list<Readback> what) {
    hipStream_t st = ctx->stream;
    for (const Readback& r : what)
      if (r.bytes) HIP_TRY(ctx, hipMemcpyAsync(r.dst, r.src, r.bytes, hipMemcpyDeviceToHost, st));
    if (poses_host && sys.nV > 0) HIP_TRY(ctx, hipMemcpyAsync(poses_host, sys.d_poses, 24 * (size_t)sys.nV, hipMemcpyDeviceToHost, st));
    HIP_TRY(ctx, hipStreamSynchronize(st));
    HIP_TRY(ctx, hipGetLastError());
    return 0;
  }
  void finish() {
    const Symbolic& S = ctx->sym;
    if (ctx->profiling) profile_collect(ctx);
    float ms = 0;
    (void)hipEventElapsedTime(&ms, ctx->ev0, ctx->ev1);
    ctx->timing[0] = S.t_order;
    ctx->timing[1] = S.t_struct;
    ctx->timing[2] = (t2 - t1) + S.t_upload;
    ctx->timing[3] = 1e-3 * ms;
    ctx->timing[4] = wall_s() - t0;
  }
};

}
```

### cg_mrslam_amd/csrc/gn_kernels.hip

```cpp
#include <hip/hip_runtime.h>
#include <stdint.h>

#include <algorithm>
#include <mutex>
#include <type_traits>

#include "gn_symbolic.h"
#include "factor_model.h"
#include "gn_device.h"
#include "gnc_device.h"
#include "init_device.h"
#include "panel_cholesky.h"
#include "switches.h"

namespace cgmr {

namespace {

constexpr int TS = 32;
constexpr unsigned long long kXSentinel = 0x7ff8c67d00000a55ull;
constexpr int kRecIntsC = (int)(sizeof(WorkRec) / 4);

#define CGMR_FRONT_CONSTS(WW)                                                                              \
  [[maybe_unused]] constexpr int W = (WW);                                                                 \
// ... 651 lines not shown
  const int lane = tid & 63, wv = tid >> 6;
  const int sa = 16 * (wv >> 1), sb = 16 * (wv & 1), lr = lane & 15, lk = lane >> 4;
  const int ri[4] = {sa + lk, sa + lk + 4, sa + lk + 8, sa + lk + 12};
  const int cj = sb + lr;
  const int gi[4] = {i0 + ri[0], i0 + ri[1], i0 + ri[2], i0 + ri[3]}, gj = j0 + cj;
  double v[MAXC][4];
  double oldv[4] = {0.0, 0.0, 0.0, 0.0};
  double* pdst[4] = {nullptr, nullptr, nullptr, nullptr};
  if (to_pan) {
#pragma unroll
    for (int q = 0; q < 4; q++) {
      const bool ok = gi[q] < r && gj <= gi[q] && gj < my_ra;
      if (ok) {
        pdst[q] = Pan + ppan + s_pp[ri[q]] + s_pp[TS + cj];
        oldv[q] = *pdst[q];
      }
    }
  }
#pragma unroll
  for (int c = 0; c < MAXC; c++)
#pragma unroll
    for (int q = 0; q < 4; q++) v[c][q] = 0.0;
  if (ncb > 0) {
#pragma unroll
  for (int c = 0; c < MAXC; c++) {
    const int cs = min(c, max(ncb - 1, 0));
    const int rg = 3 * WR->ch[cs].ns, rga = 3 * WR->ch[cs].na, nbb = rg - rga;
    const double* B = Ubuf + WR->ch[cs].U_off + (size_t)rg * even_up(rga);
    const int kj = s_k[c][TS + cj];
#pragma unroll
    for (int q = 0; q < 4; q++) {
      const int ki = s_k[c][ri[q]];
      const bool ok = c < ncb && ki >= 0 && kj >= 0 && gj <= gi[q];
      const double val = B[ok ? (size_t)(ki - rga) * nbb + (kj - rga) : 0];
      v[c][q] = ok ? val : 0.0;
    }
  }
  }
  if constexpr (MERGED) {
#pragma unroll
    for (int q = 0; q < 4; q++) {
      double cs = v[0][q];
#pragma unroll
      for (int c = 1; c < MAXC; c++) cs += v[c][q];
      v[0][q] = cs;
#pragma unroll
      for (int c = 1; c < MAXC; c++) v[c][q] = 0.0;
    }
    if (live) { LTIME_MIN(0); LTIME_MAX(2); }
    if (fresh && tid == 0) {
      const int need = max(1, (r + chunk_rows - 1) / chunk_rows);
      const int* flag = ready + rfl(WR->F.front_id);
      unsigned spins = 0;
      while (__hip_atomic_load(flag, CGMR_RLX_AGENT) < need) {
        __builtin_amdgcn_s_sleep(2);
        if (++spins > spin_limit || ((spins & 1023u) == 0 && __hip_atomic_load(status + 2, CGMR_RLX_AGENT) != 0)) {
          atomicCAS(status, 0, status[1] + 1);
          __hip_atomic_store(status + 2, 1, CGMR_RLX_AGENT);
          break;
        }
      }
    }
    __syncthreads();
    if (live) LTIME_MAX(3);
    load_slices(fresh);
    if (has_u) uval = fresh ? __longlong_as_double((long long)__hip_atomic_load((gu64*)(uvec + (size_t)3 * my_rows + pq), CGMR_RLX_AGENT)) : uvec[(size_t)3 * my_rows + pq];
    stage_slices();
    add_border_vector();
    __syncthreads();
    if (live) LTIME_MAX(4);
  }
  double4_t prod = {0.0, 0.0, 0.0, 0.0};
  {
    const double* ap = Ai + (sa + lr) * LDW + lk;
    const double* bp = Aj + (sb + lr) * LDW + lk;
    double av[W / 4], bv[W / 4];
#pragma unroll
    for (int kk = 0; kk < W / 4; kk++) { av[kk] = ap[4 * kk]; bv[kk] = bp[4 * kk]; }
#pragma unroll
    for (int kk = 0; kk < W / 4; kk++) prod = __builtin_amdgcn_mfma_f64_16x16x4f64(av[kk], bv[kk], prod, 0, 0, 0);
  }
  double acc[4] = {-prod[0], -prod[1], -prod[2], -prod[3]};
#pragma unroll
  for (int c = 0; c < (MERGED ? 1 : MAXC); c++)
#pragma unroll
    for (int q = 0; q < 4; q++) acc[q] += v[c][q];
  if constexpr (!MERGED) {
  for (int ci = MAXC; ci < nchild; ci++) {
    const FrontDesc G = fronts[children[child_off + ci]];
    const int32_t* ginv = inv + G.inv_off;
    const int rg = 3 * G.ns, rga = 3 * G.na, nbb = rg - rga;
    const double* B = Ubuf + G.U_off + (size_t)rg * even_up(rga);
    __syncthreads();
    if (tid < 2 * TS) {
      int kq = (pq < r) ? ginv[pq / 3] : -1;
      s_k[0][tid] = (short)(kq < 0 ? -1 : 3 * kq + pq % 3);
    }
    __syncthreads();
    const int kj = s_k[0][TS + cj];
#pragma unroll
    for (int q = 0; q < 4; q++) {
      const int ki = s_k[0][ri[q]];
      const bool ok = ki >= 0 && kj >= 0 && gj <= gi[q];
      acc[q] += ok ? B[(size_t)(ki - rga) * nbb + (kj - rga)] : 0.0;
    }
  }
  }
  double* Uo = Ubuf + U_off;
#pragma unroll
  for (int q = 0; q < 4; q++) {
    if (!(gi[q] < r && gj <= gi[q])) continue;
    if (pdst[q]) *pdst[q] = oldv[q] + acc[q];
    else Uo[uidx(gi[q], gj, r, my_ra)] = acc[q];
  }
  if constexpr (MERGED) { if (live) LTIME_MAX(5); }
}

template <int WW, bool BATCH>
__global__ __launch_bounds__(256) void k_front_update(const WorkRec* __restrict__ work,
                                                      const int32_t* __restrict__ tiles, int tile_begin,
                                                      const FrontDesc* __restrict__ fronts,
                                                      const int32_t* __restrict__ children,
                                                      const int32_t* __restrict__ inv, const int32_t* __restrict__ rel,
                                                      const double* __restrict__ Lbuf, double* __restrict__ Ubuf,
                                                      double* __restrict__ Pan, const double* __restrict__ uvec, long long js) {
  __shared__ UpdTileLds<WW> S;
  front_update_tile<WW, BATCH, false>(work, tiles + 3 * (size_t)(tile_begin + blockIdx.x), fronts, children, inv, rel, Lbuf, Ubuf, Pan, uvec, js,
                                      S, (int)threadIdx.x, nullptr, 0, 0, nullptr, 0u);
}

template <bool BATCH>
__global__ __launch_bounds__(kFT, 4) void k_front_level(const WorkRec* __restrict__ work, int work_begin, int nfactor, int nfactor_pad,
                                                     const double* __restrict__ PanR, double* __restrict__ Lbuf,
                                                     double* __restrict__ yvec, double* __restrict__ uvec,
                                                     int* __restrict__ status, int level_id, int write_l11c, int chunk_rows,
                                                     const int32_t* __restrict__ tiles, int tile_begin, int ntiles, int ntile_wg,
                                                     const FrontDesc* __restrict__ fronts, const int32_t* __restrict__ children,
                                                     const int32_t* __restrict__ inv, const int32_t* __restrict__ rel,
                                                     double* __restrict__ Ubuf, double* __restrict__ Pan, int* __restrict__ ready,
                                                     unsigned spin_limit, long long js) {
  extern __shared__ __attribute__((aligned(16))) unsigned char smem[];
  if ((int)blockIdx.x < nfactor_pad) {
    if ((int)blockIdx.x >= nfactor) return;
    front_factor_item<BATCH, true>(work, work_begin, PanR, Lbuf, yvec, uvec, status, level_id, write_l11c, chunk_rows, js, ready, smem);
    return;
  }
  UpdTileLds<kFrontW>* S2 = reinterpret_cast<UpdTileLds<kFrontW>*>(smem);
  const int half = (int)threadIdx.x >> 8, t = (int)blockIdx.x - nfactor_pad + half * ntile_wg;
  const int32_t* tl = t < ntiles ? tiles + 3 * (size_t)(tile_begin + t) : nullptr;
  front_update_tile<kFrontW, BATCH, true>(work, tl, fronts, children, inv, rel, Lbuf, Ubuf, Pan, uvec, js, S2[half], (int)threadIdx.x & 255,
                                          ready, level_id, chunk_rows, status, spin_limit);
}

__device__ __forceinline__ double4_t mm16(const double* X, int ldx, const double* Y, int ldy, double4_t acc, int lane) {
  const double* xp = X + (lane & 15) * ldx + (lane >> 4);
  const double* yp = Y + (lane >> 4) * ldy + (lane & 15);
#pragma unroll
  for (int kk = 0; kk < 4; kk++) acc = __builtin_amdgcn_mfma_f64_16x16x4f64(xp[4 * kk], yp[4 * kk * ldy], acc, 0, 0, 0);
  return acc;
}
__device__ __forceinline__ void st16(double* C, int ldc, double4_t v, double sign, int lane) {
#pragma unroll
  for (int rg = 0; rg < 4; rg++) C[((lane >> 4) + 4 * rg) * ldc + (lane & 15)] = sign * v[rg];
}
__device__ __forceinline__ void invert_l11_48(double* Lt, const double* dinv, double* sd, double* sp, int tid) {
  constexpr int W = 48;
  const int lane = tid & 63, wave = tid >> 6;
  if (tid < 48) {
    const int blk = tid >> 4, c = tid & 15;
    const double* D = Lt + (16 * blk) * W + 16 * blk;
    const double* di = dinv + 16 * blk;
    double z[16];
#pragma unroll
    for (int i = 0; i < 16; i++) {
      double s = 0.0;
#pragma unroll
      for (int k = 0; k < i; k++) s = fma(D[i * W + k], z[k], s);
      z[i] = (i == c ? 1.0 : -s) * di[i];
      __builtin_amdgcn_sched_barrier(0);
    }
#pragma unroll
    for (int i = 0; i < 16; i++) sd[256 * blk + 16 * i + c] = z[i];
  }
  __syncthreads();
  const double4_t zero = {0.0, 0.0, 0.0, 0.0};
  const double* A1 = sd, *C1 = sd + 256, *F1 = sd + 512;
  double* B = Lt + 16 * W, *Dm = Lt + 32 * W, *E = Lt + 32 * W + 16;
  double4_t p3 = zero;
  if (wave == 0) st16(sp, 16, mm16(B, W, A1, 16, zero, lane), 1.0, lane);
  else if (wave == 1) st16(sp + 256, 16, mm16(E, W, C1, 16, zero, lane), 1.0, lane);
  else if (wave == 2) p3 = mm16(Dm, W, A1, 16, zero, lane);
  __syncthreads();
  if (wave == 0) st16(B, W, mm16(C1, 16, sp, 16, zero, lane), -1.0, lane);
  else if (wave == 1) st16(sp + 512, 16, mm16(F1, 16, sp + 256, 16, zero, lane), -1.0, lane);
  __syncthreads();
  if (wave == 2) st16(sp, 16, mm16(E, W, B, W, p3, lane), 1.0, lane);
  __syncthreads();
  if (wave == 2) st16(Dm, W, mm16(F1, 16, sp, 16, zero, lane), -1.0, lane);
  else if (wave < 4) {
    const int t = wave == 3 ? tid - 64 : tid;
    for (int q = t; q < 256; q += 192) {
      const int i = q >> 4, j = q & 15;
      E[i * W + j] = sp[512 + q];
      Lt[i * W + j] = A1[q];
      Lt[(16 + i) * W + 16 + j] = C1[q];
      Lt[(32 + i) * W + 32 + j] = F1[q];
    }
  }
  __syncthreads();
}
template <int NT>
__device__ __forceinline__ void invert_fronts(const FrontDesc* __restrict__ fronts, int nfronts_all, int f0, int df, double* __restrict__ Lbuf, double* sm, int tid,
                                              bool top_too = false) {
  constexpr int W = 48, kDinv = 2 * W * W, kL21 = 2 * W * W + W;
  double* Lt = sm, *dinv = sm + W * W, *sd = dinv + W, *sp = sd + 768;
  for (int f = f0; f < nfronts_all; f += df) {
    if (fronts[f].pan_off < 0 && !top_too) continue;
    double* Pn = Lbuf + fronts[f].L_off;
    const int r = 3 * fronts[f].ns;
    for (int q = tid; q < W * W; q += NT) Lt[q] = Pn[q];
    if (tid < W) dinv[tid] = Pn[kDinv + tid];
    __syncthreads();
    invert_l11_48(Lt, dinv, sd, sp, tid);
    double* Z = Pn + kL21 + (size_t)r * W;
    for (int q = tid; q < W * W; q += NT) Z[q] = Lt[q];
    __syncthreads();
  }
}
constexpr int kInvertSmemBytes = (48 * 48 + 48 + 2 * 768) * 8;

constexpr int kTopPre = 32;
constexpr int kTopPreRows = 2048;
constexpr int kTopLD = kTopMaxCols + 1;
constexpr int top_smem_bytes(int ncols) {
  const int n16 = (ncols + 15) / 16 * 16;
  return ((n16 + 16) * kTopLD + n16) * 8 + kTopPreRows * 2 + kTopPre * 32;
}
static_assert(kTopMaxCols % 16 == 0 && top_smem_bytes(kTopMaxCols) <= 160 * 1024, "top block exceeds the LDS");

constexpr int kTopT = 512;
template <bool BATCH>
__global__ __launch_bounds__(kTopT) void k_top_block(int c0, int ncols, int nfronts, const int32_t* __restrict__ top_fronts,
                                                    int nchild, const int32_t* __restrict__ top_children, int nblk,
                                                    const int32_t* __restrict__ top_blocks,
                                                    const FrontDesc* __restrict__ fronts, const int32_t* __restrict__ rows,
                                                    const double* __restrict__ Ablk, const double* __restrict__ bvec,
                                                    const double* __restrict__ Ubuf, const double* __restrict__ uvec,
                                                    double* __restrict__ Lbuf, double* __restrict__ yvec,
                                                    double* __restrict__ xvec, int* __restrict__ status, int store_l,
                                                    int write_l11c, double* __restrict__ zero_ptr, long long zero_n, int nfronts_all,
                                                    int make_z, long long js) {
  CGMR_JOB(Ablk, js); CGMR_JOB(bvec, js); CGMR_JOB(Ubuf, js); CGMR_JOB(uvec, js); CGMR_JOB(Lbuf, js); CGMR_JOB(yvec, js);
  CGMR_JOB(xvec, js); CGMR_JOB(status, js); CGMR_JOB(zero_ptr, js);
  if (blockIdx.x > 0) {
    if constexpr (kFrontW == 48) {
      extern __shared__ __attribute__((aligned(16))) unsigned char smem_z[];
      if (make_z) invert_fronts<kTopT>(fronts, nfronts_all, blockIdx.x - 1, gridDim.x - 1, Lbuf, reinterpret_cast<double*>(smem_z), threadIdx.x);
    }
    if (zero_n <= 0) return;
    constexpr int H2 = kPanStride / 2;
    for (int f = blockIdx.x - 1; f < nfronts_all; f += gridDim.x - 1) {
      const long long pan_off = fronts[f].pan_off;
      if (pan_off < 0) continue;
      const int w = 3 * fronts[f].nc, r = 3 * fronts[f].ns, slots = fronts[f].pan_slots;
      const int c2n = ((w + 1) >> 1) + 1, nrow = w + r + 1;
      const long long slot2 = pan_size(fronts[f].ns) / 2;
      for (int sl = 0; sl < slots; sl++) {
        double2* z = reinterpret_cast<double2*>(zero_ptr + pan_off) + sl * slot2;
        for (int q = threadIdx.x; q < nrow * c2n; q += kTopT) {
          const int rr = q / c2n, c = q - rr * c2n;
          const int row = rr < w ? rr : kFrontW + (rr - w);
          z[row * H2 + (c < c2n - 1 ? c : kFrontW / 2)] = make_double2(0.0, 0.0);
        }
      }
    }
    return;
  }
  extern __shared__ __attribute__((aligned(16))) unsigned char smem[];
  constexpr int LD = kTopLD;
  const int n16 = (ncols + 15) / 16 * 16, M = n16 + 1, nbc = n16 / 16;
  double* P = reinterpret_cast<double*>(smem);
  double* Dinv = P + (size_t)(n16 + 16) * LD;
  short* cmap = reinterpret_cast<short*>(Dinv + n16);
  long long* ctab = reinterpret_cast<long long*>(cmap + kTopPreRows);
  const int tid = threadIdx.x, lane = tid & 63, wave = tid >> 6;
  TPHASE(0);
  const bool pre_tab = nchild <= kTopPre;
  if (pre_tab && tid < nchild) {
    const FrontDesc G = fronts[top_children[tid]];
    ctab[4 * tid] = G.U_off;
    ctab[4 * tid + 1] = (long long)(3 * G.ns) | ((long long)(3 * G.na) << 32);
    ctab[4 * tid + 2] = G.rows_off;
  }
  for (int q = tid; q < M * LD; q += kTopT) P[q] = 0.0;
  __syncthreads();
  bool pre = pre_tab;
  if (pre_tab) {
    int tot = 0;
    for (int ci = 0; ci < nchild; ci++) tot += (int)(ctab[4 * ci + 1] & 0xffffffffll);
    pre = tot <= kTopPreRows;
    if (pre) {
      int off = 0;
      for (int ci = 0; ci < nchild; ci++) {
        const int r = (int)(ctab[4 * ci + 1] & 0xffffffffll), ro = (int)ctab[4 * ci + 2];
        for (int k = tid; k < r; k += kTopT) cmap[off + k] = (short)(3 * (rows[ro + k / 3] - c0) + k % 3);
        if (tid == 0) ctab[4 * ci + 3] = off;
// ... 293 lines not shown
    BTIME(5);
    const int lane = tid & 63, wv = tid >> 6, cj = min(lane, W - 1);
    const int vi = 12 * wv + min(lane, 11);
    double v = ys[vi];
#pragma unroll
    for (int gg = 0; gg < G; gg++) v -= part[gg * W + vi];
    double s0 = 0.0, s1 = 0.0;
    const double* Zr = Lt + (12 * wv) * W + cj;
#pragma unroll
    for (int j = 0; j < 12; j += 2) {
      s0 = fma(Zr[j * W], readlane_f64(v, j), s0);
      s1 = fma(Zr[(j + 1) * W], readlane_f64(v, j + 1), s1);
    }
    if (lane < W) pz[wv * W + lane] = s0 + s1;
    BTIME(6);
    __syncthreads();
    if (tid < w) {
      const double xo = (pz[tid] + pz[W + tid]) + (pz[2 * W + tid] + pz[3 * W + tid]);
      __hip_atomic_store((gu64*)(xvec + 3 * F.c0 + tid), (unsigned long long)__double_as_longlong(xo), CGMR_RLX_AGENT);
    }
    BTIME(3);
    return;
  }
  if (tid < 64) {
    const int lane = tid;
    double v[CPL], xv[CPL];
#pragma unroll
    for (int c = 0; c < CPL; c++) {
      const int col = lane + 64 * c, cj = min(col, W - 1);
      v[c] = (col < w) ? yvec[3 * F.c0 + col] : 0.0;
#pragma unroll
      for (int gg = 0; gg < G; gg++) v[c] -= part[gg * W + cj];
      xv[c] = 0.0;
    }
    const double dv = dinv[min(lane, W - 1)];
#pragma unroll
    for (int i = W - 1; i >= 0; i--) {
      if (i < w) {
        if constexpr (LDS_L11) {
          const double xi = readlane_f64(v[i / 64], i % 64) * dinv[i];
#pragma unroll
          for (int c = 0; c < CPL; c++) {
            const int col = lane + 64 * c;
            if (col == i) xv[c] = xi;
            if (64 * c <= i) v[c] -= Lt[i * W + min(col, W - 1)] * xi;
          }
        } else {
          const double xi = readlane_f64(v[0], i) * readlane_f64(dv, i);
          if (lane == i) xv[0] = xi;
          v[0] -= Lcol[i] * xi;
        }
      }
    }
#pragma unroll
    for (int c = 0; c < CPL; c++) {
      const int col = lane + 64 * c;
      if constexpr (CHAIN) {
        if (col < w) __hip_atomic_store((gu64*)(xvec + 3 * F.c0 + col), (unsigned long long)__double_as_longlong(xv[c]), CGMR_RLX_AGENT);
      } else {
        if (col < w) xvec[3 * F.c0 + col] = xv[c];
      }
    }
  }
}

template <bool BATCH>
__global__ __launch_bounds__(256) void k_update_poses(int nV, const int32_t* __restrict__ vperm,
                                                      const uint8_t* __restrict__ cmask,
                                                      const double* __restrict__ xvec, double* __restrict__ poses,
                                                      int* __restrict__ status, long long js, long long ps) {
  CGMR_JOB(cmask, js); CGMR_JOB(xvec, js); CGMR_JOB(status, js); CGMR_JOB(poses, ps);
  int v = blockIdx.x * blockDim.x + threadIdx.x;
  if (v >= nV) return;
  const int failed = status[0];
  if (v == 0) status[1] = status[1] + 1;
  if (failed != 0) return;
  int c = vperm[v];
  if (c < 0 || cmask[c]) return;
  poses[3 * v] += xvec[3 * c];
  poses[3 * v + 1] += xvec[3 * c + 1];
  poses[3 * v + 2] = d_normalize_theta(poses[3 * v + 2] + xvec[3 * c + 2]);
}


#define CGMR_KERN(D, name) ((D).njobs > 1 ? name<true> : name<false>)

#define CGMR_LINEARIZE_TABLE(X)                                  \
  X(Ed.gnc && Ed.gnc_own_only, true, false, GncArgs)             \
  X(Ed.gnc && Ed.typed, false, false, TypedArgs, GncArgs)        \
  X(Ed.gnc, false, false, GncArgs)                               \
  X(Ed.mix && Ed.typed, false, false, TypedArgs, MixArgs)        \
  X(Ed.mix, false, false, MixArgs)                               \
  X(Ed.typed && Ed.robust, false, true, RobustArgs, TypedArgs)   \
  X(Ed.typed, false, false, TypedArgs)                           \
  X(Ed.robust && batch, true, true, RobustArgs)                  \
  X(Ed.robust, false, true, RobustArgs)                          \
  X(batch, true, false)                                          \
  X(true, false, false)

namespace {

template <typename T> const T& edge_arg(const GnEdges& Ed) {
  if constexpr (std::is_same<T, RobustArgs>::value) return Ed.rk;
  else if constexpr (std::is_same<T, TypedArgs>::value) return Ed.ty;
  else if constexpr (std::is_same<T, GncArgs>::value) return Ed.ga;
  else return Ed.mx;
}

template <bool BATCH, bool ROBUST, typename... Args>
void launch_linearize_as(hipStream_t st, const GnDevice& D, const double* poses, const GnEdges& Ed, int chi_only) {
  hipLaunchKernelGGL((k_linearize<BATCH, ROBUST, Args...>), dim3((D.nE + 255) / 256, 1, D.njobs), dim3(256), chi_only ? 0 : kRecordLds, st,
                     D.nE, Ed.nA, Ed.n_active, poses, D.ef, D.et, Ed.meas_a, Ed.info_a, Ed.meas_b, Ed.info_b, D.term, chi_only,
                     D.job_stride, D.pose_stride, edge_arg<Args>(Ed)...);
}

}

void launch_linearize(hipStream_t st, const GnDevice& D, const double* poses, const GnEdges& Ed, int chi_only) {
  if (D.nE == 0) return;
  if (Ed.chordal_stage) { launch_linearize_chordal(st, D, poses, Ed); return; }
  gn_init_kernels();
  const bool batch = D.njobs > 1;
#define CGMR_X(when, ...) if (when) return launch_linearize_as<__VA_ARGS__>(st, D, poses, Ed, chi_only);
  CGMR_LINEARIZE_TABLE(CGMR_X)
#undef CGMR_X
}

void launch_chi2(hipStream_t st, const GnDevice& D, double* out) {
  hipLaunchKernelGGL(CGMR_KERN(D, k_chi2_reduce), dim3(1, 1, D.njobs), dim3(256), 0, st, (D.nE + 255) / 256, D.term + (size_t)33 * D.nE, out, D.job_stride);
}

void launch_assemble(hipStream_t st, const GnDevice& D) {
  int total = (D.nf + D.nb) * 9 + D.nf * 3;
  hipLaunchKernelGGL(CGMR_KERN(D, k_assemble), dim3((total + 255) / 256 + 1, 1, D.njobs), dim3(256), 0, st, D.nf, D.nb, D.nE, D.asm_ptr,
                     D.asm_src, D.blk_dst, D.b_dst, D.cmask, D.off_row, D.off_col, D.term, D.Ablk, D.Pan, D.bvec, D.chi2, D.status, D.nfronts, D.xvec, D.ready, D.job_stride);
}

void launch_add_unary(hipStream_t st, const GnDevice& D, const GnEdges& Ed) {
  const UnaryLists& U = Ed.unary;
  if (!Ed.typed || U.n <= 0 || D.nf == 0) return;
  hipLaunchKernelGGL(k_add_unary, dim3((U.n * 12 + 255) / 256), dim3(256), 0, st, U.n, U.vertex, U.ptr, U.edge,
                     D.vperm, D.cmask, D.blk_dst, D.b_dst, D.term, D.Ablk, D.Pan, D.bvec);
}

void gn_init_kernels() {
  static std::once_flag once[64];
  int dev = 0;
  (void)hipGetDevice(&dev);
  std::call_once(once[dev & 63], [] {
    for (const void* f : {reinterpret_cast<const void*>(k_front_factor<false>), reinterpret_cast<const void*>(k_front_factor<true>)})
      (void)hipFuncSetAttribute(f, hipFuncAttributeMaxDynamicSharedMemorySize, factor_smem_bytes(kChunkRows + 1));
    for (const void* f : {reinterpret_cast<const void*>(k_front_level<false>), reinterpret_cast<const void*>(k_front_level<true>)})
      (void)hipFuncSetAttribute(f, hipFuncAttributeMaxDynamicSharedMemorySize, std::max(factor_smem_bytes(kChunkRows + 1), 2 * (int)sizeof(UpdTileLds<kFrontW>)));
#define CGMR_X(when, ...) reinterpret_cast<const void*>(k_linearize<__VA_ARGS__>),
    for (const void* f : {CGMR_LINEARIZE_TABLE(CGMR_X)})
#undef CGMR_X
      (void)hipFuncSetAttribute(f, hipFuncAttributeMaxDynamicSharedMemorySize, kRecordLds);
    for (const void* f : {reinterpret_cast<const void*>(k_top_block<false>), reinterpret_cast<const void*>(k_top_block<true>)})
      (void)hipFuncSetAttribute(f, hipFuncAttributeMaxDynamicSharedMemorySize, top_smem_bytes(kTopMaxCols));
  });
}

void launch_factor_level(hipStream_t st, const GnDevice& D, int l, bool write_l11c) {
  gn_init_kernels();
  int nw = D.h_work_ptr[l + 1] - D.h_work_ptr[l];
  if (nw <= 0) return;
  hipLaunchKernelGGL(CGMR_KERN(D, k_front_factor), dim3(nw, 1, D.njobs), dim3(kFT), factor_smem_bytes(D.h_level_chrows[l]), st, D.work, D.h_work_ptr[l],
                     D.Pan, D.Lbuf, D.yvec, D.uvec, D.status, l, write_l11c ? 1 : 0, D.h_level_chunk[l], D.job_stride);
}

void launch_update_level(hipStream_t st, const GnDevice& D, int l) {
  int nt = D.h_tile_ptr[l + 1] - D.h_tile_ptr[l];
  if (nt <= 0) return;
  hipLaunchKernelGGL((D.njobs > 1 ? k_front_update<kFrontW, true> : k_front_update<kFrontW, false>), dim3(nt, 1, D.njobs), dim3(256), 0, st, D.work, D.tiles, D.h_tile_ptr[l], D.fronts, D.children,
                     D.inv, D.rel, D.Lbuf, D.Ubuf, D.Pan, D.uvec, D.job_stride);
}

int level_merge_smem(const GnDevice& D, int l) { return std::max(factor_smem_bytes(D.h_level_chrows[l]), 2 * (int)sizeof(UpdTileLds<kFrontW>)); }
void launch_front_level(hipStream_t st, const GnDevice& D, int l, bool write_l11c) {
  gn_init_kernels();
  const int nw = D.h_work_ptr[l + 1] - D.h_work_ptr[l], nt = D.h_tile_ptr[l + 1] - D.h_tile_ptr[l];
  const int nw_pad = (nw + 7) / 8 * 8, ntw = ((nt + 1) / 2 + 7) / 8 * 8;
  const unsigned spin_limit = (unsigned)D.sw->bwd_spin_limit;
  hipLaunchKernelGGL(CGMR_KERN(D, k_front_level), dim3(nw_pad + ntw, 1, D.njobs), dim3(kFT), level_merge_smem(D, l), st, D.work, D.h_work_ptr[l], nw, nw_pad,
                     D.Pan, D.Lbuf, D.yvec, D.uvec, D.status, l, write_l11c ? 1 : 0, D.h_level_chunk[l], D.tiles, D.h_tile_ptr[l], nt, ntw,
                     D.fronts, D.children, D.inv, D.rel, D.Ubuf, D.Pan, D.ready, spin_limit, D.job_stride);
}
int level_merge_wgs(const GnDevice& D, int l) {
  const int nw = D.h_work_ptr[l + 1] - D.h_work_ptr[l], nt = D.h_tile_ptr[l + 1] - D.h_tile_ptr[l];
  return nt > 0 && nw > 0 ? (nw + 7) / 8 * 8 + ((nt + 1) / 2 + 7) / 8 * 8 : 0;
}
void choose_fwd_merge(GnDevice& D, int slots_div, bool off, bool any_size) {
  static int per_cu[64][4];
  static std::once_flag once[64];
  int dev = 0;
  (void)hipGetDevice(&dev);
  dev &= 63;
  gn_init_kernels();
  std::call_once(once[dev], [dev] {
    const int lds[4] = {40 * 1024, 53 * 1024, 80 * 1024, 160 * 1024};
    for (int q = 0; q < 4; q++) {
      int nb = 0;
      if (hipOccupancyMaxActiveBlocksPerMultiprocessor(&nb, reinterpret_cast<const void*>(k_front_level<false>), kFT, lds[q]) != hipSuccess) nb = 0;
      per_cu[dev][q] = std::max(0, std::min(nb, 2));
    }
  });
  int ncu = 0;
  if (hipDeviceGetAttribute(&ncu, hipDeviceAttributeMultiprocessorCount, dev) != hipSuccess) ncu = 0;
  D.h_level_merge.assign(D.nlevels, 0);
  if (!D.sw->fwd_merge || off || kFrontW != 48) return;
  for (int l = 0; l < D.nlevels; l++) {
    const int wgs = level_merge_wgs(D, l), sm = level_merge_smem(D, l);
    const int cls = sm <= 40 * 1024 ? 0 : sm <= 53 * 1024 ? 1 : sm <= 80 * 1024 ? 2 : 3;
    if (wgs > 0 && l < (int)D.h_level_mergeable.size() && D.h_level_mergeable[l] && (any_size || wgs <= per_cu[dev][cls] * ncu / std::max(1, slots_div))) D.h_level_merge[l] = 1;
  }
}

void launch_bwd_level(hipStream_t st, const GnDevice& D, int l) {
  gn_init_kernels();
  int nfr = D.h_level_ptr[l + 1] - D.h_level_ptr[l];
  if (nfr <= 0) return;
  hipLaunchKernelGGL((D.njobs > 1 ? k_solve_bwd<kFrontW, 0, true> : k_solve_bwd<kFrontW, 0, false>), dim3(nfr, 1, D.njobs), dim3(256), bwd_smem_bytes(kFrontW, false), st, D.fronts_lv, D.h_level_ptr[l], D.rows,
                     D.Lbuf, D.yvec, D.xvec, D.status, D.job_stride, 0u, 0);
}

int bwd_chain_capacity(int per_cu) {
  static int cap[64][2];
  static std::once_flag once[64];
  int dev = 0;
  (void)hipGetDevice(&dev);
  dev &= 63;
  std::call_once(once[dev], [dev] {
    int ncu = 0;
    if (hipDeviceGetAttribute(&ncu, hipDeviceAttributeMultiprocessorCount, dev) != hipSuccess) ncu = 0;
    const void* fn[2] = {reinterpret_cast<const void*>(k_solve_bwd<kFrontW, 4, false>), reinterpret_cast<const void*>(k_solve_bwd<kFrontW, 2, false>)};
    for (int q = 0; q < 2; q++) {
      int nb = 0;
      if (hipOccupancyMaxActiveBlocksPerMultiprocessor(&nb, fn[q], 256, bwd_smem_bytes(kFrontW, true)) != hipSuccess) nb = 0;
      cap[dev][q] = std::max(0, std::min(nb, q == 0 ? 4 : 2)) * ncu;
    }
  });
  return cap[dev][per_cu == 2 ? 1 : 0];
}

void launch_bwd_chain(hipStream_t st, const GnDevice& D) {
  gn_init_kernels();
  const int first = D.h_level_ptr[D.bwd_chain_level], last = D.h_level_ptr[D.nlevels];
  if (last <= first) return;
  const unsigned spin_limit = (unsigned)D.sw->bwd_spin_limit;
  auto kern = D.bwd_chain_wgs == 2 ? (D.njobs > 1 ? k_solve_bwd<kFrontW, 2, true> : k_solve_bwd<kFrontW, 2, false>)
                                   : (D.njobs > 1 ? k_solve_bwd<kFrontW, 4, true> : k_solve_bwd<kFrontW, 4, false>);
  hipLaunchKernelGGL(kern, dim3(last - first, 1, D.njobs), dim3(256), bwd_smem_bytes(kFrontW, true), st, D.fronts_lv, last - 1, D.rows,
                     D.Lbuf, D.yvec, D.xvec, D.status, D.job_stride, spin_limit, D.nlevels - 1);
}

void choose_bwd_chain(GnDevice& D, int slots_div, bool levelwise) {
  const int chain_env = D.sw->bwd_chain, wgs_env = D.sw->bwd_chain_wgs;
  slots_div = std::max(1, slots_div);
  const int total = D.h_level_ptr[D.nlevels] - D.h_level_ptr[0];
  int cap2 = bwd_chain_capacity(2) / slots_div, cap4 = bwd_chain_capacity(4) / slots_div;
  if (chain_env >= 0) { cap2 = std::min(cap2, chain_env); cap4 = std::min(cap4, chain_env); }
  D.bwd_chain_wgs = wgs_env == 2 || wgs_env == 4 ? wgs_env : (total <= cap2 ? 2 : 4);
  const int cap = D.bwd_chain_wgs == 2 ? cap2 : cap4;
  D.bwd_chain_level = D.nlevels;
  while (!levelwise && D.bwd_chain_level > 0 && D.h_level_ptr[D.nlevels] - D.h_level_ptr[D.bwd_chain_level - 1] <= cap) D.bwd_chain_level--;
}

void launch_top_block(hipStream_t st, const GnDevice& D, bool store_l, bool write_l11c, bool clear_panels, bool make_z) {
  gn_init_kernels();
  if (D.top_nfronts <= 0) return;
  const bool zero = clear_panels && D.pan_doubles > 0;
  make_z = make_z && kFrontW == 48;
  hipLaunchKernelGGL(CGMR_KERN(D, k_top_block), dim3(zero || make_z ? 1 + 240 : 1, 1, D.njobs), dim3(kTopT), std::max(top_smem_bytes(D.top_ncols), kInvertSmemBytes), st, D.top_c0, D.top_ncols,
                     D.top_nfronts, D.top_fronts, D.top_nchild, D.top_children, D.top_nblk, D.top_blocks, D.fronts, D.rows, D.Ablk,
                     D.bvec, D.Ubuf, D.uvec, D.Lbuf, D.yvec, D.xvec, D.status, store_l ? 1 : 0, write_l11c ? 1 : 0, D.Pan,
                     zero ? (long long)D.pan_doubles : 0ll, D.nfronts, make_z ? 1 : 0, D.job_stride);
}

void launch_invert_fronts(hipStream_t st, const GnDevice& D, bool top_too) {
  if (kFrontW != 48 || D.nfronts <= 0) return;
  hipLaunchKernelGGL(CGMR_KERN(D, k_invert_fronts), dim3(std::min(D.nfronts, 512), 1, D.njobs), dim3(256), kInvertSmemBytes, st, D.fronts, D.nfronts, D.Lbuf, D.job_stride,
                     top_too ? 1 : 0);
}

void launch_update(hipStream_t st, const GnDevice& D, double* poses) {
  hipLaunchKernelGGL(CGMR_KERN(D, k_update_poses), dim3((D.nV + 255) / 256, 1, D.njobs), dim3(256), 0, st, D.nV, D.vperm, D.cmask, D.xvec, poses,
                     D.status, D.job_stride, D.pose_stride);
}

}

#ifdef CGMR_PHASE_TIMING
extern "C" int cgmr_debug_topphase(unsigned long long* out) {
  return (int)hipMemcpyFromSymbol(out, HIP_SYMBOL(cgmr::g_tphase), sizeof(unsigned long long) * 16);
}
extern "C" int cgmr_debug_leveltimes(unsigned long long* out, int reset) {
  if (reset) {
    unsigned long long z[8 * 64];
    for (int l = 0; l < 64; l++) { z[8 * l] = ~0ull; for (int q = 1; q < 8; q++) z[8 * l + q] = 0; }
    return (int)hipMemcpyToSymbol(HIP_SYMBOL(cgmr::g_ltime), z, sizeof z);
  }
  return (int)hipMemcpyFromSymbol(out, HIP_SYMBOL(cgmr::g_ltime), sizeof(unsigned long long) * 8 * 64);
}
extern "C" int cgmr_debug_bwdtimes(unsigned long long* out) {
  return (int)hipMemcpyFromSymbol(out, HIP_SYMBOL(cgmr::g_btime), sizeof(unsigned long long) * 8 * 8192);
}
extern "C" int cgmr_debug_workphases(unsigned long long* out) {
  return (int)hipMemcpyFromSymbol(out, HIP_SYMBOL(cgmr::g_wphase), sizeof(unsigned long long) * 8 * 8192);
}
extern "C" int cgmr_debug_factorphases(unsigned long long* out) {
  return (int)hipMemcpyFromSymbol(out, HIP_SYMBOL(cgmr::g_fphase), sizeof(unsigned long long) * 8 * 8192);
}
extern "C" int cgmr_debug_worktimes(unsigned long long* out) {
  return (int)hipMemcpyFromSymbol(out, HIP_SYMBOL(cgmr::g_wtime), sizeof(unsigned long long) * 2 * 8192);
}
extern "C" int cgmr_debug_phase(unsigned long long* out) {
  return (int)hipMemcpyFromSymbol(out, HIP_SYMBOL(cgmr::g_phase), sizeof(unsigned long long) * 64 * 8);
}
#endif
```

### cg_mrslam_amd/csrc/gn_symbolic.h

```cpp
#pragma once
#include <functional>
#include <cstdint>
#include <vector>

namespace cgmr {

struct Switches;

#ifndef CGMR_PANEL_POSES
#define CGMR_PANEL_POSES 16
#endif
constexpr int kPanelW = CGMR_PANEL_POSES;
constexpr int kFrontW = (3 * kPanelW + 15) / 16 * 16;
constexpr int64_t factor_header(int w) { return 2 * (int64_t)w * w + w; }
constexpr int kChunkRows = (kFrontW <= 48 ? 208 : 192) - kFrontW - 1;
constexpr int kMidChunkRows = 79;

constexpr int kTopChunkRows = 31;
constexpr int kTopChunkFronts = 8;
constexpr int kLeafChunkRows = 95;

constexpr int kTopMaxCols = 128;

constexpr int kSmallSlabLoads = 4;
constexpr bool slab_is_small(int ns, int na) {
  const int cpw = (3 * na + 1) / 2 > 1 ? (3 * na + 1) / 2 : 1;
  const int rows = (256 / cpw) * kSmallSlabLoads < 256 ? (256 / cpw) * kSmallSlabLoads : 256;
  return 3 * ns <= rows;
}

struct FrontDesc {
  int32_t c0;
  int32_t nc;
  int32_t ns;
  int32_t rows_off;
  int32_t parent;
  int32_t level;
  int32_t child_off;
  int32_t nchild;
  int32_t rel_off;
  int32_t na;
  int32_t inv_off;
  int32_t a_off;
  int32_t a_cnt;
  int32_t pan_slots;
  int64_t L_off;
  int64_t U_off;
  int64_t pan_off;
  int64_t ppan_off;
  int32_t p_nc, p_ns;
  int32_t sched_t;
  int32_t sched_slot;
  int32_t front_id;
  int32_t p_c0;
};
constexpr int kPanStride = kFrontW + 2;
constexpr int64_t pan_size(int ns) { return (int64_t)(kFrontW + 3 * ns + 1) * kPanStride; }
constexpr int kMaxPanSlots = 3;

constexpr int kWorkChildren = 8;
struct WorkChild {
  int64_t U_off;
  int32_t ns, na;
  int32_t rel_off, inv_off, rows_off;
  int32_t pad;
};
struct WorkRec {
  FrontDesc F;
  int32_t front, chunk, pad[2];
  WorkChild ch[kWorkChildren];
};
static_assert(sizeof(WorkChild) == 32 && sizeof(WorkRec) % 8 == 0, "WorkRec layout");

struct Symbolic {
  int nV = 0, nE = 0;
  int nf = 0;
  int nb = 0;
  std::vector<int32_t> hidx;
  std::vector<int32_t> vperm;
  std::vector<int32_t> perm;
  int64_t n_rel = 0, n_inv = 0;
  std::vector<int32_t> off_row, off_col;
  std::vector<FrontDesc> fronts;
  std::vector<int32_t> rows, children;
  std::vector<int32_t> level_ptr;
  std::vector<int32_t> level_fronts;
  std::vector<int32_t> col_front;
  std::vector<int32_t> top_fronts;
  int32_t top_c0 = 0, top_nposes = 0;
  std::vector<int32_t> top_children;
  std::vector<int32_t> top_blocks;
  std::vector<int32_t> gn_level_ptr, gn_level_fronts;
  int64_t L_doubles = 0, U_doubles = 0, pan_doubles = 0;
  struct NDNode { int32_t parent = -1, a = -1, b = -1, count = 0; std::vector<int32_t> verts; };
  std::vector<NDNode> nd_nodes;
  int32_t nd_root = -1;
  struct NDRecLite { int32_t a, b, n, ssz; };
  std::vector<NDRecLite> nd_pending_recs;
  std::vector<int32_t> nd_pending_order, nd_pending_hubs;
  int32_t nd_pending_root = -1;
  bool nd_pending = false;
  int32_t nd_nf_full = 0;
  int32_t nd_appended = 0;
  int32_t nd_height_full = 0;
  bool extended = false;
  int max_ns = 0;
  double flops = 0;
  double t_order = 0, t_struct = 0;
  double t_upload = 0;
};

void host_run_tasks(int n, const std::function<void(int)>& task);

struct AnalyzeHooks {
  std::function<int(const Symbolic&, const int32_t* offbase)> blocks_ready;
};
int analyze(int nV, const uint8_t* fixed, int nE, const int32_t* ef, const int32_t* et, Symbolic& S, const Switches& sw, Symbolic* prev = nullptr,
            int n_common = -1, const int32_t* hub_vertices = nullptr, int n_hub_vertices = 0, const AnalyzeHooks* hooks = nullptr);

struct StructureRef {
  std::vector<int32_t> asm_ptr;
  std::vector<int32_t> asm_src;
  std::vector<int32_t> rel, inv;
  std::vector<int32_t> blk_dst;
  std::vector<int32_t> b_dst;
};
int structure_reference(const Symbolic& S, int nE, const int32_t* ef, const int32_t* et, StructureRef& R);

}
```

### cg_mrslam_amd/csrc/switches.h

```cpp
#pragma once
#include <algorithm>
#include <cstdio>
#include <cstdlib>

#include "gn_symbolic.h"

namespace cgmr {

#define CGMR_SWITCH_TABLE(X)                                                                                                        \
                                                                                                    \
  X("CGMR_FWD_MERGE", fwd_merge, flag, true, context, "a level's factorisation and update tiles in one launch where it is certainly resident; 0: two launches per level") \
  X("CGMR_FWD_MERGE_ANY", fwd_merge_any, flag, true, context, "merged level launches also where residency is not certain, until the context's first time-out; 0: never") \
  X("CGMR_BWD_CHAIN", bwd_chain, num, -1, context, "at most n workgroups in the chained backward solve; 0: one launch per level; -1: what is certainly resident") \
  X("CGMR_BWD_CHAIN_WGS", bwd_chain_wgs, num, 0, context, "2 / 4: that instance of the chained backward solve (workgroups per CU); else chosen by tree size") \
  X("CGMR_BWD_SPIN_LIMIT", bwd_spin_limit, min1, 1 << 22, context, "polls a bounded device-side wait may take (chained backward solve, merged levels) before it times out") \
  X("CGMR_TOP_BLOCK", top_block, flag, true, context, "the last fronts of the root's chain in one launch (k_top_block); 0: fronts like any other") \
  X("CGMR_CLEAR_IN_TOP", clear_in_top, flag, true, context, "the top-block launch clears the panels for the next pass; 0: a memset per pass") \
  X("CGMR_CHUNK", mid_chunk, chunk, kMidChunkRows, context, "border rows per work item above the leaves") \
  X("CGMR_LEAF_CHUNK", leaf_chunk, chunk, kLeafChunkRows, context, "border rows per work item on a level of leaves") \
  X("CGMR_TOP_CHUNK", top_chunk, chunk, kTopChunkRows, context, "border rows per work item on a level of at most CGMR_TOP_CHUNK_FRONTS fronts") \
  X("CGMR_TOP_CHUNK_FRONTS", top_chunk_fronts, num, kTopChunkFronts, context, "fronts a level may have to take CGMR_TOP_CHUNK") \
  X("CGMR_GRAPH", graph, flag, false, context, "capture one Gauss-Newton iteration into a hipGraph and replay it")                 \
                                                                                                                      \
  X("CGMR_AMALGAMATE", amalgamate, flag, true, context, "merge a front into its parent where that is free; 0: one front per panel")  \
  X("CGMR_ND_REUSE_START", nd_reuse_start, flag, true, context, "a dissection node starts its sweep where the parent's ended; 0: its own far-vertex sweep") \
  X("CGMR_ND_ROOT_STARTS", nd_root_starts, num, 4, context, "structuring sweeps the root runs side by side (at most 16); 0 / 1: the double sweep") \
  X("CGMR_ND_INHERIT", nd_inherit, flag, true, context, "a dissection node takes the sweep its caller already holds (near half, first component); 0: it sweeps anew") \
  X("CGMR_ND_MIN_COVER", nd_min_cover, flag, true, context, "separator = minimum vertex cover between two levels; 0: the whole level") \
  X("CGMR_ND_PAR_DEPTH", nd_par_depth, num, -1, context, "dissection levels that fork a helper thread; -1: by the number of host threads") \
  X("CGMR_HUB_DEGREE", hub_degree, num, 32, context, "vertices of more neighbours are eliminated last (hubs); 0: no hubs, named ones included") \
  X("CGMR_SYM_EXTEND", sym_extend, flag, true, context, "a grown graph extends the cached ordering; 0: every analysis from scratch")  \
  X("CGMR_SYM_EXTEND_CHECK", sym_extend_check, flag, true, context, "an extension checks that new edges keep subtrees independent; 0: unchecked (a known-wrong structure)") \
  X("CGMR_SYM_EXTEND_SLACK", sym_extend_slack, num, 2, context, "panels an extended tree may be taller than the last from-scratch one; negative: no bound") \
  X("CGMR_ADJ_SLICES", adj_slices, flag, true, context, "adjacency built from per-thread slices of the edge list; 0: per-thread vertex ranges") \
                                                                                                  \
  X("CGMR_MATCH_EDT", match_edt, flag, true, context, "rasterise by a distance transform where the kernel table allows it; 0: stamp the kernel per point") \
  X("CGMR_MATCH_SPLIT", match_split, min1, 16, context, "workgroups that may share one pair's search angles")                       \
  X("CGMR_MATCH_PRUNE", match_prune, flag, true, context, "drop candidates that cannot win when the bin count is not asked for; 0: score them all") \
  X("CGMR_MATCH_LEAN", match_lean, flag, true, context, "lean kernel instances for the usual batch shape, the general one behind them; 0: the general one only") \
  X("CGMR_MATCH_NOREDO", match_noredo, flag, false, context, "profiling only: pairs the lean instance hands back are not searched (their results are wrong)") \
  X("CGMR_HIER_HOST", hier_host, flag, false, context, "hierarchical search level by level from the host; default: the levels chained on the device") \
  X("CGMR_GUESS_CACHED", guess_cached, flag, true, context, "condensed graphs: initial guess by the cached spanning-tree walk; 0: the general edge-list walk") \
                                                                                                               \
  X("CGMR_TRACE_LAUNCHES", trace_launches, set, false, context, "name every solver launch and synchronise after it")                \
  X("CGMR_GN_TRACE", gn_trace, set, false, context, "where a solve's wall time goes, summed, printed when the context is destroyed") \
  X("CGMR_SYM_TRACE", sym_trace, set, false, context, "the analysis' phases, one line each")                                        \
  X("CGMR_COND_TRACE", cond_trace, set, false, context, "the condensed-graph batch's phases")                                       \
  X("CGMR_MATCH_TRACE", match_trace, set, false, context, "the generic searches' stages, one line each")                            \
                                                                                    \
  X("CGMR_HOST_THREADS", host_threads, num, 0, process, "threads of an analysis, caller included (at most 16); 0: by CPU count and cgroup quota") \
  X("CGMR_HOST_PIN", host_pin, num, 1, process, "1: a helper per core around the creating CPU's cache group; 2: anywhere in that group; 0: not pinned") \
  X("CGMR_HOST_PIN_CALLER", host_pin_caller, flag, false, process, "hold the calling thread on the pool's home core while it analyses") \
  X("CGMR_HOST_MOVE", host_move, flag, false, process, "move the pool to another cache group when its cores are kept busy by others") \
  X("CGMR_HOST_STEAL", host_steal, flag, true, process, "a waiting caller runs its own queued jobs; 0: it only waits")                 \
  X("CGMR_HOST_SPIN_US", host_spin_us, min0, 200, process, "microseconds an idle helper spins before it sleeps")                    \
  X("CGMR_RCCL_LIB", rccl_lib, text, nullptr, process, "path of the RCCL library to load when the default names are not found")

namespace switch_kind {
typedef bool flag; typedef bool set;
typedef int num; typedef int chunk; typedef int min0; typedef int min1;
typedef const char* text;
}

struct Switches {
#define X(var, field, kind, def, scope, effect) switch_kind::kind field = def;
  CGMR_SWITCH_TABLE(X)
#undef X
};

namespace switch_parse {
inline bool flag(const char* e) { return atoi(e) != 0; }
inline bool set(const char*) { return true; }
inline int num(const char* e) { return atoi(e); }
inline int chunk(const char* e) { return std::min(kChunkRows, std::max(16, atoi(e))); }
inline int min0(const char* e) { return std::max(0, atoi(e)); }
inline int min1(const char* e) { return std::max(1, atoi(e)); }
inline const char* text(const char* e) { return e; }
}

inline Switches read_switches() {
  Switches s;
#define X(var, field, kind, def, scope, effect) if (const char* e = getenv(var)) s.field = switch_parse::kind(e);
  CGMR_SWITCH_TABLE(X)
#undef X
  return s;
}

inline const Switches& process_switches() {
  static const Switches s = read_switches();
  return s;
}

inline int list_switches(const Switches& ctx_sw, const Switches& proc_sw, char* buf, int cap) {
  struct Put {
    static int value(char* b, size_t n, bool v) { return snprintf(b, n, "%d", v ? 1 : 0); }
    static int value(char* b, size_t n, int v) { return snprintf(b, n, "%d", v); }
    static int value(char* b, size_t n, const char* v) { return snprintf(b, n, "%s", v ? v : ""); }
  };
  const Switches &context = ctx_sw, &process = proc_sw;
  size_t need = 0;
  auto room = [&](char*& at) { at = need < (size_t)std::max(cap, 0) ? buf + need : nullptr; return at ? (size_t)cap - need : 0; };
  char* at;
  size_t n;
#define X(var, field, kind, def, scope, effect)                         \
  n = room(at); need += snprintf(at, n, "%s\t%s\t", var, #scope);       \
  n = room(at); need += Put::value(at, n, scope.field);                 \
  n = room(at); need += snprintf(at, n, "\t%s\n", effect);
  CGMR_SWITCH_TABLE(X)
#undef X
  return (int)need + 1;
}

}
```

### include/cgmr.h

```cpp
#ifndef CGMR_H
#define CGMR_H

#include <stddef.h>
#include <stdint.h>

#ifdef __cplusplus
extern "C" {
#endif

#define CGMR_OK 0
#define CGMR_E_INVALID (-1)
#define CGMR_E_NO_DEVICE (-2)
#define CGMR_E_HIP (-3)
#define CGMR_E_ALLOC (-4)
#define CGMR_E_TIMEOUT (-5)
#define CGMR_E_CHOLESKY_BASE (-100)

typedef struct cgmr_ctx cgmr_ctx;

int cgmr_version(void);

int cgmr_ctx_create(int device, void* hip_stream, cgmr_ctx** out);
void cgmr_ctx_destroy(cgmr_ctx* ctx);
const char* cgmr_last_error(const cgmr_ctx* ctx);
// ... 68 lines not shown
#define CGMR_DL_STEP_DL 3
int cgmr_dl_optimize(cgmr_ctx* ctx, int nV, double* poses_xyt, const uint8_t* fixed, int nE, const int32_t* from_idx,
                     const int32_t* to_idx, const double* meas_xyt, const double* info_upper, int iters,
                     const cgmr_dl_params* params, double* chi2_out, double* delta_out, int32_t* trials_out,
                     int32_t* step_out, int32_t* iters_done, const cgmr_robust* rk);
int cgmr_dl_optimize_dev(cgmr_ctx* ctx, int nV, double* d_poses_xyt, const uint8_t* fixed, int nE,
                         const int32_t* from_idx, const int32_t* to_idx, const double* d_meas_xyt,
                         const double* d_info_upper, int iters, const cgmr_dl_params* params, double* chi2_out,
                         double* delta_out, int32_t* trials_out, int32_t* step_out, int32_t* iters_done,
                         const cgmr_robust* rk);
int cgmr_dl_last_stats(const cgmr_ctx* ctx, int64_t out[3]);

#define CGMR_VERTEX_SE2 0
#define CGMR_VERTEX_XY 1
#define CGMR_EDGE_SE2 0
#define CGMR_EDGE_SE2_XY 1
#define CGMR_EDGE_BEARING_SE2_XY 2
#define CGMR_EDGE_PRIOR_SE2 3
#define CGMR_EDGE_PRIOR_SE2_XY 4
typedef struct cgmr_factor_types {
  const uint8_t* vertex_kind;
  const uint8_t* edge_kind;
} cgmr_factor_types;
int cgmr_gn_optimize_typed(cgmr_ctx* ctx, int nV, double* poses_xyt, const uint8_t* fixed, int nE, const int32_t* from_idx,
                           const int32_t* to_idx, const double* meas_xyt, const double* info_upper, int iters,
                           double* chi2_out, const cgmr_factor_types* types, const cgmr_robust* rk);
int cgmr_gn_optimize_typed_dev(cgmr_ctx* ctx, int nV, double* d_poses_xyt, const uint8_t* fixed, int nE,
                               const int32_t* from_idx, const int32_t* to_idx, const double* d_meas_xyt,
                               const double* d_info_upper, int iters, double* chi2_out, const cgmr_factor_types* types,
                               const cgmr_robust* rk);
int cgmr_lm_optimize_typed(cgmr_ctx* ctx, int nV, double* poses_xyt, const uint8_t* fixed, int nE, const int32_t* from_idx,
                           const int32_t* to_idx, const double* meas_xyt, const double* info_upper, int iters,
                           const cgmr_lm_params* params, double* chi2_out, double* lambda_out, int32_t* trials_out,
                           int32_t* iters_done, const cgmr_factor_types* types, const cgmr_robust* rk);
int cgmr_lm_optimize_typed_dev(cgmr_ctx* ctx, int nV, double* d_poses_xyt, const uint8_t* fixed, int nE,
                               const int32_t* from_idx, const int32_t* to_idx, const double* d_meas_xyt,
                               const double* d_info_upper, int iters, const cgmr_lm_params* params, double* chi2_out,
                               double* lambda_out, int32_t* trials_out, int32_t* iters_done,
                               const cgmr_factor_types* types, const cgmr_robust* rk);
int cgmr_dl_optimize_typed(cgmr_ctx* ctx, int nV, double* poses_xyt, const uint8_t* fixed, int nE, const int32_t* from_idx,
                           const int32_t* to_idx, const double* meas_xyt, const double* info_upper, int iters,
                           const cgmr_dl_params* params, double* chi2_out, double* delta_out, int32_t* trials_out,
                           int32_t* step_out, int32_t* iters_done, const cgmr_factor_types* types, const cgmr_robust* rk);
int cgmr_dl_optimize_typed_dev(cgmr_ctx* ctx, int nV, double* d_poses_xyt, const uint8_t* fixed, int nE,
                               const int32_t* from_idx, const int32_t* to_idx, const double* d_meas_xyt,
                               const double* d_info_upper, int iters, const cgmr_dl_params* params, double* chi2_out,
                               double* delta_out, int32_t* trials_out, int32_t* step_out, int32_t* iters_done,
                               const cgmr_factor_types* types, const cgmr_robust* rk);
typedef struct cgmr_mixture {
  const int32_t* comp_ptr;
  const double* comp_meas;
  const double* comp_info;
  const double* comp_weight;
  int32_t* selected_out;
} cgmr_mixture;
int cgmr_gn_optimize_mixture(cgmr_ctx* ctx, int nV, double* poses_xyt, const uint8_t* fixed, int nE, const int32_t* from_idx,
                             const int32_t* to_idx, const double* meas_xyt, const double* info_upper, int iters,
                             double* chi2_out, const cgmr_factor_types* types, const cgmr_mixture* mixture);
int cgmr_gn_optimize_mixture_dev(cgmr_ctx* ctx, int nV, double* d_poses_xyt, const uint8_t* fixed, int nE,
                                 const int32_t* from_idx, const int32_t* to_idx, const double* d_meas_xyt,
                                 const double* d_info_upper, int iters, double* chi2_out, const cgmr_factor_types* types,
                                 const cgmr_mixture* mixture);
int cgmr_lm_optimize_mixture(cgmr_ctx* ctx, int nV, double* poses_xyt, const uint8_t* fixed, int nE, const int32_t* from_idx,
                             const int32_t* to_idx, const double* meas_xyt, const double* info_upper, int iters,
                             const cgmr_lm_params* params, double* chi2_out, double* lambda_out, int32_t* trials_out,
                             int32_t* iters_done, const cgmr_factor_types* types, const cgmr_mixture* mixture);
int cgmr_lm_optimize_mixture_dev(cgmr_ctx* ctx, int nV, double* d_poses_xyt, const uint8_t* fixed, int nE,
                                 const int32_t* from_idx, const int32_t* to_idx, const double* d_meas_xyt,
                                 const double* d_info_upper, int iters, const cgmr_lm_params* params, double* chi2_out,
                                 double* lambda_out, int32_t* trials_out, int32_t* iters_done,
                                 const cgmr_factor_types* types, const cgmr_mixture* mixture);
int cgmr_dl_optimize_mixture(cgmr_ctx* ctx, int nV, double* poses_xyt, const uint8_t* fixed, int nE, const int32_t* from_idx,
                             const int32_t* to_idx, const double* meas_xyt, const double* info_upper, int iters,
                             const cgmr_dl_params* params, double* chi2_out, double* delta_out, int32_t* trials_out,
                             int32_t* step_out, int32_t* iters_done, const cgmr_factor_types* types,
                             const cgmr_mixture* mixture);
int cgmr_dl_optimize_mixture_dev(cgmr_ctx* ctx, int nV, double* d_poses_xyt, const uint8_t* fixed, int nE,
                                 const int32_t* from_idx, const int32_t* to_idx, const double* d_meas_xyt,
                                 const double* d_info_upper, int iters, const cgmr_dl_params* params, double* chi2_out,
                                 double* delta_out, int32_t* trials_out, int32_t* step_out, int32_t* iters_done,
                                 const cgmr_factor_types* types, const cgmr_mixture* mixture);
int cgmr_mixture_select(cgmr_ctx* ctx, int nV, const double* poses_xyt, const uint8_t* fixed, int nE, const int32_t* from_idx,
                        const int32_t* to_idx, const double* meas_xyt, const double* info_upper,
                        const cgmr_factor_types* types, const cgmr_mixture* mixture, double* chi2_out);
#define CGMR_GNC_TLS 0
#define CGMR_GNC_GM 1
typedef struct cgmr_gnc_params {
  int32_t loss;
  double mu_factor;
  int32_t max_outer;
  int32_t inner_iters;
  int32_t outer_per_wait;
  const double* barc_sq;
  double default_barc_sq;
  const uint8_t* known_inlier;
  double* weight_out;
  double* edge_chi2_out;
} cgmr_gnc_params;
cgmr_gnc_params cgmr_gnc_params_default(void);
int cgmr_gnc_optimize(cgmr_ctx* ctx, int nV, double* poses_xyt, const uint8_t* fixed, int nE, const int32_t* from_idx,
                      const int32_t* to_idx, const double* meas_xyt, const double* info_upper, const cgmr_factor_types* types,
                      const cgmr_gnc_params* params, double* mu_out, double* cost_out, int32_t* partial_out, int32_t* outer_done);
int cgmr_gnc_optimize_dev(cgmr_ctx* ctx, int nV, double* d_poses_xyt, const uint8_t* fixed, int nE, const int32_t* from_idx,
                          const int32_t* to_idx, const double* d_meas_xyt, const double* d_info_upper,
                          const cgmr_factor_types* types, const cgmr_gnc_params* params, double* mu_out, double* cost_out,
                          int32_t* partial_out, int32_t* outer_done);
int cgmr_gnc_last_stats(const cgmr_ctx* ctx, int64_t out[2]);
#define CGMR_CHORDAL_ROTATION 1
#define CGMR_CHORDAL_TRANSLATION 2
int cgmr_chordal_initialize(cgmr_ctx* ctx, int nV, double* poses_xyt, const uint8_t* fixed, int nE, const int32_t* from_idx,
                            const int32_t* to_idx, const double* meas_xyt, const double* info_upper, int stages,
                            double* chi2_out, int32_t* counts_out);
int cgmr_chordal_initialize_dev(cgmr_ctx* ctx, int nV, double* d_poses_xyt, const uint8_t* fixed, int nE,
                                const int32_t* from_idx, const int32_t* to_idx, const double* d_meas_xyt,
                                const double* d_info_upper, int stages, double* chi2_out, int32_t* counts_out);
int cgmr_chordal_initialize_typed(cgmr_ctx* ctx, int nV, double* poses_xyt, const uint8_t* fixed, int nE,
                                  const int32_t* from_idx, const int32_t* to_idx, const double* meas_xyt,
                                  const double* info_upper, int stages, double* chi2_out, int32_t* counts_out,
                                  const cgmr_factor_types* types);
int cgmr_chordal_initialize_typed_dev(cgmr_ctx* ctx, int nV, double* d_poses_xyt, const uint8_t* fixed, int nE,
                                      const int32_t* from_idx, const int32_t* to_idx, const double* d_meas_xyt,
                                      const double* d_info_upper, int stages, double* chi2_out, int32_t* counts_out,
                                      const cgmr_factor_types* types);
int cgmr_initial_guess(int nV, double* poses_xyt, const uint8_t* fixed, int nE, const int32_t* from_idx, const int32_t* to_idx,
                       const double* meas_xyt);
int cgmr_marginals_typed(cgmr_ctx* ctx, int nV, const double* poses_xyt, const uint8_t* fixed, int nE,
                         const int32_t* from_idx, const int32_t* to_idx, const double* meas_xyt, const double* info_upper,
                         int nK, const int32_t* query_idx, double* cov_out, const cgmr_factor_types* types,
                         const cgmr_robust* rk);
int cgmr_marginals_all_typed(cgmr_ctx* ctx, int nV, const double* poses_xyt, const uint8_t* fixed, int nE,
                             const int32_t* from_idx, const int32_t* to_idx, const double* meas_xyt,
                             const double* info_upper, double* cov_out, double* cross_out,
                             const cgmr_factor_types* types, const cgmr_robust* rk);

int cgmr_set_symbolic_cache(cgmr_ctx* ctx, int on);
int cgmr_symbolic_cache_stats(const cgmr_ctx* ctx, int64_t out[2]);
int cgmr_symbolic_cache_stats3(const cgmr_ctx* ctx, int64_t out[3]);
int64_t cgmr_gn_timeouts(const cgmr_ctx* ctx);
int cgmr_switches(const cgmr_ctx* ctx_or_null, char* buf, int cap);

int cgmr_host_threads_info(int32_t out[5]);

int cgmr_gn_symbolic_info(int nV, const uint8_t* fixed, int nE, const int32_t* from_idx,
                          const int32_t* to_idx, int64_t out[16], int32_t* perm_out);

int cgmr_gn_symbolic_info_grown(int nV0, int nE0, int n_steps, const int32_t* nV_step, const int32_t* nE_step,
                                const int32_t* from_idx, const int32_t* to_idx, int64_t out[16], int32_t* perm_out,
                                int32_t* n_extended_out);

int cgmr_gn_last_timing(const cgmr_ctx* ctx, double out[5]);

int cgmr_set_profiling(cgmr_ctx* ctx, int on);
int cgmr_gn_kernel_times(const cgmr_ctx* ctx, double seconds_out[8], int64_t launches_out[8]);
int cgmr_gn_kernel_times_ex(const cgmr_ctx* ctx, double seconds_out[12], int64_t launches_out[12]);

typedef struct cgmr_matcher_config {
  float grid_ll_x, grid_ll_y, grid_ur_x, grid_ur_y;
  double resolution;
  double kernel_range;
  int kscale;
  double win_x, win_y, win_theta;
  double theta_res;
  double bin_x, bin_y, bin_theta;
  double subsample_res;
  int n_beams;
  double angle_min, angle_inc, max_range, min_range;
  double laser_pose[3];
} cgmr_matcher_config;

void cgmr_matcher_config_close(cgmr_matcher_config* cfg, int n_beams, double angle_min, double angle_inc,
                               double max_range);

int cgmr_match_close_batch(cgmr_ctx* ctx, const cgmr_matcher_config* cfg, int n_pairs, const float* ranges_ref,
                           const float* ranges_qry, const double* guess_xyt, double max_score, double* out_xyt,
                           double* out_score, uint8_t* out_found, int32_t* out_nresults);
int cgmr_match_close_batch_dev(cgmr_ctx* ctx, const cgmr_matcher_config* cfg, int n_pairs,
                               const float* d_ranges_ref, const float* d_ranges_qry, const double* d_guess_xyt,
                               double max_score, double* d_out_xyt, double* d_out_score, uint8_t* d_out_found,
                               int32_t* d_out_nresults);
int cgmr_match_close_vset_batch(cgmr_ctx* ctx, const cgmr_matcher_config* cfg, int n_pairs, int n_ref_scans,
                                const float* ranges_ref, const double* ref_rel_xyt, const float* ranges_qry,
                                const double* guess_xyt, double max_score, double* out_xyt, double* out_score,
                                uint8_t* out_found, int32_t* out_nresults);
int cgmr_match_close_vset_batch_dev(cgmr_ctx* ctx, const cgmr_matcher_config* cfg, int n_pairs, int n_ref_scans,
                                    const float* d_ranges_ref, const double* d_ref_xform, const float* d_ranges_qry,
                                    const double* d_guess_xyt, double max_score, double* d_out_xyt, double* d_out_score,
                                    uint8_t* d_out_found, int32_t* d_out_nresults);
int cgmr_scan_transforms(const cgmr_matcher_config* cfg, int n, const double* rel_xyt, double* xform_out);
int cgmr_match_last_stats(const cgmr_ctx* ctx, int64_t out[2]);
int cgmr_match_last_redo_pairs(const cgmr_ctx* ctx, int64_t* out);
int cgmr_match_last_path_counts(const cgmr_ctx* ctx, int64_t out[4]);
int cgmr_match_last_launch_shape(const cgmr_ctx* ctx, int64_t out[4]);
int cgmr_match_last_kernel_seconds(const cgmr_ctx* ctx, double* seconds);

int cgmr_marginals(cgmr_ctx* ctx, int nV, const double* poses_xyt, const uint8_t* fixed, int nE,
                   const int32_t* from_idx, const int32_t* to_idx, const double* meas_xyt, const double* info_upper,
                   int nK, const int32_t* query_idx, double* cov_out);
int cgmr_marginals_all(cgmr_ctx* ctx, int nV, const double* poses_xyt, const uint8_t* fixed, int nE,
                       const int32_t* from_idx, const int32_t* to_idx, const double* meas_xyt,
                       const double* info_upper, double* cov_out, double* cross_out);
int cgmr_covariance_estimate(cgmr_ctx* ctx, int nV, const double* poses_xyt, int nE, const int32_t* from_idx,
                             const int32_t* to_idx, const double* meas_xyt, const double* info_upper, int gauge_idx,
                             int nK, const int32_t* query_idx, double* cov_out);
int cgmr_condense(cgmr_ctx* ctx, int nV, const double* poses_xyt, int nE, const int32_t* from_idx,
                  const int32_t* to_idx, const double* meas_xyt, const double* info_upper, int gauge_idx, int nK,
                  const int32_t* query_idx, int32_t* to_out, double* est_out, double* info_upper_out, double* cov_out);
int cgmr_marginals_robust(cgmr_ctx* ctx, int nV, const double* poses_xyt, const uint8_t* fixed, int nE,
                          const int32_t* from_idx, const int32_t* to_idx, const double* meas_xyt, const double* info_upper,
                          int nK, const int32_t* query_idx, double* cov_out, const cgmr_robust* rk);
int cgmr_marginals_all_robust(cgmr_ctx* ctx, int nV, const double* poses_xyt, const uint8_t* fixed, int nE,
                              const int32_t* from_idx, const int32_t* to_idx, const double* meas_xyt,
                              const double* info_upper, double* cov_out, double* cross_out, const cgmr_robust* rk);
int cgmr_covariance_estimate_robust(cgmr_ctx* ctx, int nV, const double* poses_xyt, int nE, const int32_t* from_idx,
                                    const int32_t* to_idx, const double* meas_xyt, const double* info_upper, int gauge_idx,
                                    int nK, const int32_t* query_idx, double* cov_out, const cgmr_robust* rk);
int cgmr_condense_robust(cgmr_ctx* ctx, int nV, const double* poses_xyt, int nE, const int32_t* from_idx,
                         const int32_t* to_idx, const double* meas_xyt, const double* info_upper, int gauge_idx, int nK,
                         const int32_t* query_idx, int32_t* to_out, double* est_out, double* info_upper_out, double* cov_out,
                         const cgmr_robust* rk);

#define CGMR_JOINT_MAX_QUERIES 2048
int cgmr_marginals_joint(cgmr_ctx* ctx, int nV, const double* poses_xyt, const uint8_t* fixed, int nE,
                         const int32_t* from_idx, const int32_t* to_idx, const double* meas_xyt, const double* info_upper,
                         int nK, const int32_t* query_idx, double* cov_out, const cgmr_robust* rk);
int cgmr_marginals_pairs(cgmr_ctx* ctx, int nV, const double* poses_xyt, const uint8_t* fixed, int nE,
                         const int32_t* from_idx, const int32_t* to_idx, const double* meas_xyt, const double* info_upper,
                         int nP, const int32_t* pair_a, const int32_t* pair_b, double* cov_aa_out, double* cov_ab_out,
                         double* cov_bb_out, const cgmr_robust* rk);
int cgmr_relative_covariance(cgmr_ctx* ctx, int nV, const double* poses_xyt, const uint8_t* fixed, int nE,
                             const int32_t* from_idx, const int32_t* to_idx, const double* meas_xyt, const double* info_upper,
                             int nP, const int32_t* pair_a, const int32_t* pair_b, double* rel_xyt_out, double* rel_cov_out,
                             const double* hyp_meas_xyt, const double* hyp_info_upper, double* d2_out, const cgmr_robust* rk);

int cgmr_marginals_joint_typed(cgmr_ctx* ctx, int nV, const double* poses_xyt, const uint8_t* fixed, int nE,
                               const int32_t* from_idx, const int32_t* to_idx, const double* meas_xyt,
                               const double* info_upper, int nK, const int32_t* query_idx, double* cov_out,
                               const cgmr_factor_types* types, const cgmr_robust* rk);
int cgmr_marginals_pairs_typed(cgmr_ctx* ctx, int nV, const double* poses_xyt, const uint8_t* fixed, int nE,
                               const int32_t* from_idx, const int32_t* to_idx, const double* meas_xyt,
                               const double* info_upper, int nP, const int32_t* pair_a, const int32_t* pair_b,
                               double* cov_aa_out, double* cov_ab_out, double* cov_bb_out, const cgmr_factor_types* types,
                               const cgmr_robust* rk);
int cgmr_observation_covariance(cgmr_ctx* ctx, int nV, const double* poses_xyt, const uint8_t* fixed, int nE,
                                const int32_t* from_idx, const int32_t* to_idx, const double* meas_xyt,
                                const double* info_upper, int nP, const int32_t* pair_a, const int32_t* pair_b,
                                const uint8_t* obs_kind, double* z_out, double* cov_out, const double* hyp_meas_xyt,
                                const double* hyp_info_upper, double* d2_out, const cgmr_factor_types* types,
                                const cgmr_robust* rk);

#define CGMR_PCM_MAX_CLOSURES 1024
int cgmr_closure_consistency(cgmr_ctx* ctx, int nV, const double* poses_xyt, const uint8_t* fixed, int nE,
                             const int32_t* from_idx, const int32_t* to_idx, const double* meas_xyt, const double* info_upper,
                             int nC, const int32_t* cl_a, const int32_t* cl_b, const double* cl_meas_xyt,
                             const double* cl_info_upper, double gamma, double* d2_out, uint64_t* adj_out,
                             int32_t* clique_out, int32_t* clique_size_out, int32_t* seed_out, const cgmr_robust* rk);
int cgmr_max_clique_greedy(cgmr_ctx* ctx, int n, const uint64_t* adj_bits, int32_t* clique_out, int32_t* clique_size_out,
                           int32_t* seed_out);

#define CGMR_EXACT_DEFAULT_NODE_LIMIT 512
int cgmr_closure_consistency_exact(cgmr_ctx* ctx, int nV, const double* poses_xyt, const uint8_t* fixed, int nE,
                                   const int32_t* from_idx, const int32_t* to_idx, const double* meas_xyt,
                                   const double* info_upper, int nC, const int32_t* cl_a, const int32_t* cl_b,
                                   const double* cl_meas_xyt, const double* cl_info_upper, double gamma, double* d2_out,
                                   uint64_t* adj_out, int64_t node_limit, int32_t* clique_out, int32_t* clique_size_out,
                                   int32_t* proven_out, const cgmr_robust* rk);
int cgmr_max_clique_exact(cgmr_ctx* ctx, int n, const uint64_t* adj_bits, int64_t node_limit, int32_t* clique_out,
                          int32_t* clique_size_out, int32_t* proven_out, int64_t* nodes_out);

int cgmr_closure_consistency_inter(cgmr_ctx* ctx, int nV, const double* poses_xyt, const uint8_t* fixed, int nE,
                                   const int32_t* from_idx, const int32_t* to_idx, const double* meas_xyt,
                                   const double* info_upper, int nC, const int32_t* cl_a, const double* peer_pose_xyt,
                                   const double* peer_cov, const double* cl_meas_xyt, const double* cl_info_upper, double gamma,
                                   double* d2_out, uint64_t* adj_out, int32_t* clique_out, int32_t* clique_size_out,
                                   int32_t* seed_out, const cgmr_robust* rk);
int cgmr_closure_consistency_inter_exact(cgmr_ctx* ctx, int nV, const double* poses_xyt, const uint8_t* fixed, int nE,
                                         const int32_t* from_idx, const int32_t* to_idx, const double* meas_xyt,
                                         const double* info_upper, int nC, const int32_t* cl_a, const double* peer_pose_xyt,
                                         const double* peer_cov, const double* cl_meas_xyt, const double* cl_info_upper,
                                         double gamma, double* d2_out, uint64_t* adj_out, int64_t node_limit,
                                         int32_t* clique_out, int32_t* clique_size_out, int32_t* proven_out,
                                         const cgmr_robust* rk);

typedef struct cgmr_match_result { double x, y, theta, score; } cgmr_match_result;
int cgmr_match_greedy(cgmr_ctx* ctx, const cgmr_matcher_config* cfg, int n_ref, const double* ref_pts_xy, int n_qry,
                      const double* qry_pts_xy, int n_regions, const float* regions, double step_x, double step_y,
                      double theta_res, double max_score, double dx, double dy, double dth,
                      cgmr_match_result* results_out, int cap, int* n_out);

typedef struct cgmr_scan_set {
  int n_scans;
  const float* ranges;
  const double* poses_xyt;
  int ref_index;
} cgmr_scan_set;
int cgmr_close_scan_matching(cgmr_ctx* ctx, const cgmr_matcher_config* cfg, const cgmr_scan_set* vset,
                             const float* cur_ranges, const double cur_pose_xyt[3], double max_score, double trel_out[3],
                             int* found_out);
int cgmr_scan_matching_lc(cgmr_ctx* ctx, const cgmr_matcher_config* cfg, const cgmr_scan_set* ref_set,
                          const cgmr_scan_set* cur_set, double max_score, double* trel_out, int* n_out);
int cgmr_global_matching(cgmr_ctx* ctx, const cgmr_matcher_config* cfg, const cgmr_scan_set* ref_set,
                         const cgmr_scan_set* cur_set, double max_score, double trel_out[3], int* found_out);
int cgmr_scan_matching_lc_hierarchical(cgmr_ctx* ctx, const cgmr_matcher_config* cfg, const cgmr_scan_set* ref_set,
                                       const cgmr_scan_set* cur_set, double max_score, double trel_out[3], int* found_out);
int cgmr_verify_matching(cgmr_ctx* ctx, const cgmr_matcher_config* cfg, const cgmr_scan_set* set1, const cgmr_scan_set* set2,
                         const double trel12[3], double* score_out, int* accepted_out);
int cgmr_match_hierarchical(cgmr_ctx* ctx, const cgmr_matcher_config* cfg, int n_ref, const double* ref_pts_xy, int n_qry,
                            const double* qry_pts_xy, int n_regions, const float* regions, double theta_res, double max_score,
// ... 205 lines not shown
```

Before: 2004 GN iterations/s.

## Add self-sufficient update tiles for small merged levels to avoid intra-launch waits

For non-leaf merged levels with at most a configurable number of update tiles, a new kernel variant has each update tile redo the panel Cholesky of its front's rows itself. It no longer spins waiting for the factorisation workgroup in the same launch. This removes the ready-flag synchronisation and the residency concerns of the merged launch on small upper levels. The cost is redundant factorisation work per tile, extra LDS, and a new per-tile descriptor array. The feature is on by default (threshold 128 tiles).

```diff
diff --git a/cg_mrslam_amd/_lib.py b/cg_mrslam_amd/_lib.py
--- a/cg_mrslam_amd/_lib.py
+++ b/cg_mrslam_amd/_lib.py
@@ -922,15 +922,23 @@
         self._check(self.lib.cgmr_set_profiling(self.h, C.c_int(1 if on else 0)))
 
     def gn_kernel_times(self):
-        sec = np.zeros(12)
-        n = np.zeros(12, dtype=np.int64)
+        sec = np.zeros(13)
+        n = np.zeros(13, dtype=np.int64)
         self._check(self.lib.cgmr_gn_kernel_times_ex(self.h, _ptr(sec), _ptr(n)))
         names = ["linearize", "assemble", "chi2", "front_factor", "front_update", "top_block", "solve_bwd", "update", "front_level"]
-        return {k: (float(s), int(c)) for k, s, c in zip(names, sec, n)}
+        out = {k: (float(s), int(c)) for k, s, c in zip(names, sec, n)}
+        out["front_level"] = (float(sec[8] + sec[12]), int(n[8] + n[12]))
+        return out
+
+    def self_level_times(self):
+        sec = np.zeros(13)
+        n = np.zeros(13, dtype=np.int64)
+        self._check(self.lib.cgmr_gn_kernel_times_ex(self.h, _ptr(sec), _ptr(n)))
+        return float(sec[12]), int(n[12])
 
     def pcm_kernel_times(self):
-        sec = np.zeros(12)
-        n = np.zeros(12, dtype=np.int64)
+        sec = np.zeros(13)
+        n = np.zeros(13, dtype=np.int64)
         self._check(self.lib.cgmr_gn_kernel_times_ex(self.h, _ptr(sec), _ptr(n)))
         return {k: (float(sec[i]), int(n[i])) for i, k in zip((9, 10, 11), ("gram", "consistency", "bits_clique"))}
 
diff --git a/cg_mrslam_amd/csrc/cgmr_api.cpp b/cg_mrslam_amd/csrc/cgmr_api.cpp
--- a/cg_mrslam_amd/csrc/cgmr_api.cpp
+++ b/cg_mrslam_amd/csrc/cgmr_api.cpp
@@ -864,11 +864,11 @@
   return CGMR_OK;
 }
 
-extern "C" int cgmr_gn_kernel_times_ex(const cgmr_ctx* ctx, double seconds_out[12], int64_t launches_out[12]) {
+extern "C" int cgmr_gn_kernel_times_ex(const cgmr_ctx* ctx, double seconds_out[13], int64_t launches_out[13]) {
   if (!ctx || !seconds_out || !launches_out) return CGMR_E_INVALID;
-  memcpy(seconds_out, ctx->ksec, sizeof(double) * 12);
-  memcpy(launches_out, ctx->klaunch, sizeof(int64_t) * 12);
-  return CGMR_OK;
-}
-
-}
+  memcpy(seconds_out, ctx->ksec, sizeof(double) * 13);
+  memcpy(launches_out, ctx->klaunch, sizeof(int64_t) * 13);
+  return CGMR_OK;
+}
+
+}
diff --git a/cg_mrslam_amd/csrc/cgmr_ctx.h b/cg_mrslam_amd/csrc/cgmr_ctx.h
--- a/cg_mrslam_amd/csrc/cgmr_ctx.h
+++ b/cg_mrslam_amd/csrc/cgmr_ctx.h
@@ -79,8 +79,8 @@
   int64_t match_shape[4] = {0, 0, 0, 0};
   int64_t match_redo_pairs = 0;
   bool profiling = false;
-  double ksec[12] = {0};
-  int64_t klaunch[12] = {0};
+  double ksec[13] = {0};
+  int64_t klaunch[13] = {0};
   std::vector<hipEvent_t> ev_pool;
   std::vector<int> ev_cls;
   hipEvent_t ev0 = nullptr, ev1 = nullptr, ev_a = nullptr, ev_b = nullptr;
diff --git a/cg_mrslam_amd/csrc/gn_device.h b/cg_mrslam_amd/csrc/gn_device.h
--- a/cg_mrslam_amd/csrc/gn_device.h
+++ b/cg_mrslam_amd/csrc/gn_device.h
@@ -43,6 +43,10 @@
   std::vector<int32_t> h_level_chunk;
   std::vector<uint8_t> h_level_mergeable;
   std::vector<uint8_t> h_level_merge;
+  std::vector<uint8_t> h_level_self;
+  int32_t* tiles_x = nullptr;
+  std::vector<int32_t> h_tilex_ptr;
+  std::vector<int32_t> h_level_ntiles;
   std::vector<int32_t> h_level_chrows;
 };
 
@@ -102,6 +106,7 @@
 void launch_factor_level(hipStream_t st, const GnDevice& D, int level, bool write_l11c);
 void launch_update_level(hipStream_t st, const GnDevice& D, int level);
 void launch_front_level(hipStream_t st, const GnDevice& D, int level, bool write_l11c);
+void launch_front_level_self(hipStream_t st, const GnDevice& D, int level, bool write_l11c);
 void choose_fwd_merge(GnDevice& D, int slots_div, bool off, bool any_size = false);
 void launch_bwd_level(hipStream_t st, const GnDevice& D, int level);
 void launch_bwd_chain(hipStream_t st, const GnDevice& D);
diff --git a/cg_mrslam_amd/csrc/gn_host.cpp b/cg_mrslam_amd/csrc/gn_host.cpp
--- a/cg_mrslam_amd/csrc/gn_host.cpp
+++ b/cg_mrslam_amd/csrc/gn_host.cpp
@@ -160,6 +160,8 @@
   D.h_level_leaf.assign(D.nlevels, 1);
   D.h_level_chunk.assign(D.nlevels, kChunkRows);
   D.h_level_mergeable.assign(D.nlevels, 1);
+  D.h_level_ntiles.assign(D.nlevels, 0);
+  D.h_tilex_ptr.assign(D.nlevels + 1, 0);
   std::vector<std::vector<int32_t>> sched(D.nlevels);
   for (int q = 0; q < (int)LF.size(); q++) {
     const FrontDesc& F = S.fronts[LF[q]];
@@ -188,8 +190,12 @@
       if (S.fronts[f].nchild > kWorkChildren) D.h_level_mergeable[l] = 0;
       const int T = (3 * S.fronts[f].ns + 31) / 32;
       *std::min_element(xload, xload + 8) += T * (T + 1) / 2;
+      D.h_level_ntiles[l] += T * (T + 1) / 2;
     }
     D.h_tile_ptr[l + 1] = D.h_tile_ptr[l] + 8 * *std::max_element(xload, xload + 8);
+    const bool self_tiles_candidate = sw.fwd_merge && !D.h_level_leaf[l] && D.h_level_mergeable[l] && D.h_level_ntiles[l] > 0 &&
+                                      D.h_level_ntiles[l] <= sw.fwd_self_tiles;
+    D.h_tilex_ptr[l + 1] = D.h_tilex_ptr[l] + (self_tiles_candidate ? D.h_tile_ptr[l + 1] - D.h_tile_ptr[l] : 0);
     D.h_work_ptr[l + 1] = D.h_work_ptr[l] + nwork;
   }
   const size_t n_tiles = (size_t)D.h_tile_ptr[D.nlevels], n_work = (size_t)D.h_work_ptr[D.nlevels];
@@ -200,6 +206,7 @@
   size_t o_children = B.add<int32_t>(S.children.size());
   size_t o_lf = B.add<int32_t>(S.level_fronts.size());
   size_t o_tiles = B.add<int32_t>(3 * n_tiles);
+  size_t o_tilex = B.add<int32_t>((size_t)kSelfTileInts * D.h_tilex_ptr[D.nlevels] + 4);
   size_t o_rec0 = B.add<int32_t>(rec0_of.size());
   size_t o_tf = B.add<int32_t>(S.top_fronts.size()), o_tc = B.add<int32_t>(S.top_children.size()), o_tb = B.add<int32_t>(S.top_blocks.size());
   size_t blob_bytes = (B.off + 255) & ~size_t(255);
@@ -236,14 +243,23 @@
           int32_t* tl = tiles + 3 * (size_t)D.h_tile_ptr[l];
           const int slots = D.h_tile_ptr[l + 1] - D.h_tile_ptr[l];
           for (int k = 0; k < slots; k++) { tl[3 * k] = -1; tl[3 * k + 1] = 0; tl[3 * k + 2] = 0; }
+          int32_t* tx = D.h_tilex_ptr[l + 1] > D.h_tilex_ptr[l] ? reinterpret_cast<int32_t*>(h + o_tilex) + (size_t)kSelfTileInts * D.h_tilex_ptr[l] : nullptr;
+          if (tx) for (int k = 0; k < slots; k++) { tx[kSelfTileInts * k] = -1; for (int q = 1; q < kSelfTileInts; q++) tx[kSelfTileInts * k + q] = 0; }
           int xload[8] = {0, 0, 0, 0, 0, 0, 0, 0};
           for (int f : sched[l]) {
             const int T = (3 * S.fronts[f].ns + 31) / 32;
             const int x = (int)(std::min_element(xload, xload + 8) - xload);
             for (int ti = 0; ti < T; ti++)
               for (int tj = 0; tj <= ti; tj++) {
-                int32_t* e = tl + 3 * (size_t)(8 * xload[x]++ + x);
+                const size_t slot = (size_t)(8 * xload[x]++ + x);
+                int32_t* e = tl + 3 * slot;
                 e[0] = rec0_of[2 * f]; e[1] = ti; e[2] = tj;
+                if (tx) {
+                  const FrontDesc& F = S.fronts[f];
+                  int32_t* ex = tx + kSelfTileInts * slot;
+                  ex[0] = e[0]; ex[1] = ti; ex[2] = tj; ex[3] = F.nc; ex[4] = F.ns; ex[5] = F.pan_slots;
+                  ex[6] = (int32_t)(uint32_t)((uint64_t)F.pan_off & 0xffffffffu); ex[7] = (int32_t)(F.pan_off >> 32);
+                }
               }
           }
         }
@@ -289,6 +305,7 @@
   D.b_dst = (int32_t*)(d + o_rdst);
   D.level_fronts = (int32_t*)(d + o_lf);
   D.tiles = (int32_t*)(d + o_tiles);
+  D.tiles_x = (int32_t*)(d + o_tilex);
   D.work = (WorkRec*)(d + o_work);
   D.asm_ptr = V.asm_ptr; D.asm_src = V.asm_src; D.vperm = V.vperm; D.ef = V.ef; D.et = V.et; D.off_row = V.off_row; D.off_col = V.off_col;
   D.cmask = (uint8_t*)(d + o_cmask);
@@ -459,6 +476,7 @@
       fprintf(stderr, "[cgmr] level %d: %d fronts, %d work items, max r %d, max child rows %d\n", l,
               D.h_level_ptr[l + 1] - D.h_level_ptr[l], D.h_work_ptr[l + 1] - D.h_work_ptr[l], maxr, maxc);
     }
+    if (l < (int)D.h_level_self.size() && D.h_level_self[l]) { T.run(12, 1, [&] { launch_front_level_self(st, D, l, write_l11c); }); continue; }
     if (l < (int)D.h_level_merge.size() && D.h_level_merge[l]) { T.run(8, 1, [&] { launch_front_level(st, D, l, write_l11c); }); continue; }
     T.run(3, 1, [&] { launch_factor_level(st, D, l, write_l11c); });
     if (D.h_tile_ptr[l + 1] > D.h_tile_ptr[l]) T.run(4, 1, [&] { launch_update_level(st, D, l); });
@@ -485,6 +503,8 @@
   merge_was = D.h_level_merge;
   D.bwd_chain_level = D.nlevels;
   D.h_level_merge.assign(D.nlevels, 0);
+  self_was = D.h_level_self;
+  D.h_level_self.assign(D.nlevels, 0);
   const int fresh[4] = {0, it0, 0, 0};
   HIP_TRY(ctx, hipMemcpyAsync(D.status, fresh, sizeof fresh, hipMemcpyHostToDevice, st));
   return 0;
diff --git a/cg_mrslam_amd/csrc/gn_host.h b/cg_mrslam_amd/csrc/gn_host.h
--- a/cg_mrslam_amd/csrc/gn_host.h
+++ b/cg_mrslam_amd/csrc/gn_host.h
@@ -66,7 +66,7 @@
   GnDevice& D;
   bool armed = false;
   int chain_was = 0;
-  std::vector<uint8_t> merge_was;
+  std::vector<uint8_t> merge_was, self_was;
   LevelwiseScope(cgmr_ctx* c, GnDevice& d) : ctx(c), D(d) {}
   LevelwiseScope(const LevelwiseScope&) = delete;
   LevelwiseScope& operator=(const LevelwiseScope&) = delete;
@@ -75,6 +75,7 @@
     if (!armed) return;
     D.bwd_chain_level = chain_was;
     D.h_level_merge.swap(merge_was);
+    D.h_level_self.swap(self_was);
   }
 };
 struct GnSystem {
@@ -123,7 +124,7 @@
   template <typename Fn>
   void run(int cls, int nlaunch, Fn&& fn) {
     if (ctx->sw.trace_launches) {
-      fprintf(stderr, "[cgmr] launch class %d (0 lin 1 asm 2 chi2 3 factor 4 update 5 top 6 bwd 7 poses 8 factor+update)\n", cls);
+      fprintf(stderr, "[cgmr] launch class %d (0 lin 1 asm 2 chi2 3 factor 4 update 5 top 6 bwd 7 poses 8 factor+update 12 factor+self-sufficient tiles)\n", cls);
       fn();
       hipError_t e = hipStreamSynchronize(st);
       fprintf(stderr, "[cgmr]   done: %s\n", hipGetErrorString(e));
diff --git a/cg_mrslam_amd/csrc/gn_kernels.hip b/cg_mrslam_amd/csrc/gn_kernels.hip
--- a/cg_mrslam_amd/csrc/gn_kernels.hip
+++ b/cg_mrslam_amd/csrc/gn_kernels.hip
@@ -827,6 +827,214 @@
                                           ready, level_id, chunk_rows, status, spin_limit);
 }
 
+constexpr int kSelfPanelRows = (kFrontW + 2 * TS + 1 + 15) / 16 * 16;
+template <int WW>
+struct SelfTileLds {
+  double P[kSelfPanelRows * (WW + 1)];
+  double Dinv[WW];
+  short s_k[MAXC][2 * TS];
+  int s_pp[2 * TS];
+};
+static_assert(sizeof(SelfTileLds<kFrontW>) == (kSelfPanelRows * (kFrontW + 1) + kFrontW) * 8 + MAXC * 2 * TS * 2 + 2 * TS * 4, "self-sufficient tile: LDS plan");
+static_assert(sizeof(SelfTileLds<kFrontW>) <= 64 * 1024, "self-sufficient tile: LDS plan exceeds 64 KiB");
+static_assert(kFrontW + 2 * TS + 1 <= 16 + kElimRows * (kFT / 64), "panel_cholesky: at most 8 x 48 rows below a diagonal block");
+constexpr int kSelfRPP = kFT / (kPanStride / 2);
+constexpr int kSelfLoads = (kFrontW + 2 * TS + 1 + kSelfRPP - 1) / kSelfRPP;
+template <int WW, bool BATCH>
+__device__ __forceinline__ void front_update_tile_self(const WorkRec* __restrict__ work, const int32_t* __restrict__ tl,
+                                                       const int32_t* __restrict__ inv, const int32_t* __restrict__ rel,
+                                                       const double* __restrict__ PanR, double* __restrict__ Ubuf,
+                                                       double* __restrict__ Pan, long long js, SelfTileLds<WW>& S, int level_id) {
+  CGMR_JOB(PanR, js); CGMR_JOB(Ubuf, js); CGMR_JOB(Pan, js);
+  CGMR_FRONT_CONSTS(WW);
+  static_assert(WW == kFrontW, "the assembled panels are laid out for kFrontW columns");
+  double* P = S.P;
+  auto& s_k = S.s_k;
+  int* s_pp = S.s_pp;
+  const int tid = threadIdx.x;
+  const int rec = rfl(tl[0]);
+  if (rec < 0) return;
+  const int ti = rfl(tl[1]), tj = rfl(tl[2]);
+  const int w = 3 * rfl(tl[3]), ns = rfl(tl[4]), r = 3 * ns, slots = rfl(tl[5]);
+  const long long pan_off = ((long long)rfl(tl[7]) << 32) | (unsigned)rfl(tl[6]);
+  LTIME_MIN(0);
+  const WorkRec* WR = work + rec;
+  const int my_ra = 3 * rfl(WR->F.na), nchild = rfl(WR->F.nchild);
+  const long long U_off = rfl64(WR->F.U_off), ppan = rfl64(WR->F.ppan_off);
+  const int p_w = 3 * rfl(WR->F.p_nc), p_r = 3 * rfl(WR->F.p_ns), my_rel = rfl(WR->F.rel_off);
+  const int ncb = min(nchild, MAXC);
+  const int i0 = ti * TS, j0 = tj * TS;
+  const bool two = tj != ti;
+  const int RH = W + (two ? 2 * TS : TS), M = RH + 1;
+  const bool to_pan = ppan >= 0 && j0 < my_ra;
+  const bool tw = tid < 256;
+  int kb[MAXC];
+  int myrel = 0;
+  const int pq = (tid < TS) ? i0 + tid : j0 + tid - TS;
+  constexpr int H2 = kPanStride / 2;
+  const int pc = tid % H2, prow0 = tid / H2, c2 = 2 * pc;
+  const bool tact = prow0 < kSelfRPP;
+  const bool colneed = tact && (c2 < ((w + 1) & ~1) || c2 == W);
+  double2 pv[kSelfLoads];
+  {
+    const double2* src = reinterpret_cast<const double2*>(PanR + pan_off);
+    const size_t slot2 = (size_t)pan_size(ns) / 2;
+    double2 pv1[kSelfLoads];
+    int so[kSelfLoads];
+    bool need[kSelfLoads];
+#pragma unroll
+    for (int u = 0; u < kSelfLoads; u++) {
+      const int row = prow0 + kSelfRPP * u;
+      const int b = row < W + TS ? i0 + row - W : j0 + row - W - TS;
+      so[u] = (row < W ? row : (row < RH ? W + b : W + r)) * H2 + pc;
+      need[u] = colneed && row < M && !(row >= w && row < W) && !(row >= W && row < RH && b >= r);
+      pv[u] = need[u] ? src[so[u]] : make_double2(0.0, 0.0);
+    }
+#pragma unroll
+    for (int c = 0; c < MAXC; c++) {
+      const int cs = min(c, max(ncb - 1, 0));
+      kb[c] = (tid < 2 * TS && pq < r && c < ncb) ? inv[WR->ch[cs].inv_off + pq / 3] : -1;
+    }
+    myrel = (ppan >= 0 && tid < 2 * TS && pq < r) ? rel[my_rel + pq / 3] : 0;
+    if (slots > 1) {
+#pragma unroll
+      for (int u = 0; u < kSelfLoads; u++) pv1[u] = need[u] ? src[slot2 + so[u]] : make_double2(0.0, 0.0);
+#pragma unroll
+      for (int u = 0; u < kSelfLoads; u++) { pv[u].x += pv1[u].x; pv[u].y += pv1[u].y; }
+      for (int sl = 2; sl < slots; sl++) {
+#pragma unroll
+        for (int u = 0; u < kSelfLoads; u++) pv1[u] = need[u] ? src[sl * slot2 + so[u]] : make_double2(0.0, 0.0);
+#pragma unroll
+        for (int u = 0; u < kSelfLoads; u++) { pv[u].x += pv1[u].x; pv[u].y += pv1[u].y; }
+      }
+    }
+  }
+  asm volatile("" : "+v"(myrel));
+  if (tid < 2 * TS) {
+#pragma unroll
+    for (int c = 0; c < MAXC; c++) s_k[c][tid] = (short)(kb[c] < 0 ? -1 : 3 * kb[c] + pq % 3);
+    const int pos = 3 * myrel + pq % 3;
+    s_pp[tid] = tid < TS ? (pos < p_w ? pos : W + pos - p_w) * kPanStride : pos;
+  }
+  const bool has_u = ppan >= 0 && tj == 0 && tid < TS && pq < r;
+#pragma unroll
+  for (int u = 0; u < kSelfLoads; u++) {
+    const int row = prow0 + kSelfRPP * u;
+    if (!tact || row >= M) continue;
+    double vx = pv[u].x, vy = pv[u].y;
+    if (row >= w && row < W) {
+      if (c2 == row) vx = 1.0;
+      if (c2 + 1 == row) vy = 1.0;
+    }
+    P[row * LDW + c2] = vx;
+    if (c2 + 1 < LDW) P[row * LDW + c2 + 1] = vy;
+  }
+  __syncthreads();
+  LTIME_MAX(2);
+  double* udst = nullptr;
+  double uold = 0.0;
+  {
+    const int pos = 3 * myrel + pq % 3;
+    udst = has_u ? Pan + ppan + (pos < p_w ? (size_t)(W + p_r) * kPanStride + pos : (size_t)(W + pos - p_w) * kPanStride + W) : nullptr;
+    if (ppan >= 0 && tj == 0 && tid < TS) uold = *(has_u ? udst : Pan + ppan);
+  }
+  const int lane = tid & 63, wv = tid >> 6;
+  const int sa = 16 * ((wv >> 1) & 1), sb = 16 * (wv & 1), lr = lane & 15, lk = lane >> 4;
+  const int ri[4] = {sa + lk, sa + lk + 4, sa + lk + 8, sa + lk + 12};
+  const int cj = sb + lr;
+  const int gi[4] = {i0 + ri[0], i0 + ri[1], i0 + ri[2], i0 + ri[3]}, gj = j0 + cj;
+  double v[MAXC][4];
+  double oldv[4] = {0.0, 0.0, 0.0, 0.0};
+  double* pdst[4] = {nullptr, nullptr, nullptr, nullptr};
+  unsigned vok = 0u;
+  if (tw && to_pan) {
+#pragma unroll
+    for (int q = 0; q < 4; q++) {
+      const bool ok = gi[q] < r && gj <= gi[q] && gj < my_ra;
+      pdst[q] = ok ? Pan + ppan + s_pp[ri[q]] + s_pp[TS + cj] : nullptr;
+      oldv[q] = *(ok ? pdst[q] : Pan + ppan);
+    }
+  }
+#pragma unroll
+  for (int c = 0; c < MAXC; c++)
+#pragma unroll
+    for (int q = 0; q < 4; q++) v[c][q] = 0.0;
+  if (tw && ncb > 0) {
+#pragma unroll
+    for (int c = 0; c < MAXC; c++) {
+      const int cs = min(c, max(ncb - 1, 0));
+      const int rg = 3 * WR->ch[cs].ns, rga = 3 * WR->ch[cs].na, nbb = rg - rga;
+      const double* B = Ubuf + WR->ch[cs].U_off + (size_t)rg * even_up(rga);
+      const int kj = s_k[c][TS + cj];
+#pragma unroll
+      for (int q = 0; q < 4; q++) {
+        const int ki = s_k[c][ri[q]];
+        const bool ok = c < ncb && ki >= 0 && kj >= 0 && gj <= gi[q];
+        v[c][q] = B[ok ? (size_t)(ki - rga) * nbb + (kj - rga) : 0];
+        vok |= ok ? 1u << (4 * c + q) : 0u;
+      }
+    }
+  }
+  auto roff = [](int row) -> int { return row * LDW; };
+  const int nbc = min(W / 16, (w + 15) >> 4);
+  (void)panel_cholesky<kFT / 64>(P, roff, M, nbc, S.Dinv, lane, wv);
+  LTIME_MAX(3);
+  if (!tw) return;
+  if (has_u) {
+    const double* xr = P + (W + tid) * LDW;
+    const double* yr = P + RH * LDW;
+    double dot = 0.0;
+#pragma unroll 8
+    for (int k = 0; k < W; k++) dot = fma(xr[k], yr[k], dot);
+    *udst = uold + (xr[W] - dot);
+  }
+  double4_t prod = {0.0, 0.0, 0.0, 0.0};
+  {
+    const double* Ai = P + W * LDW;
+    const double* Aj = two ? P + (W + TS) * LDW : Ai;
+    const double* ap = Ai + (sa + lr) * LDW + lk;
+    const double* bp = Aj + (sb + lr) * LDW + lk;
+    double av[W / 4], bv[W / 4];
+#pragma unroll
+    for (int kk = 0; kk < W / 4; kk++) { av[kk] = ap[4 * kk]; bv[kk] = bp[4 * kk]; }
+#pragma unroll
+    for (int kk = 0; kk < W / 4; kk++) prod = __builtin_amdgcn_mfma_f64_16x16x4f64(av[kk], bv[kk], prod, 0, 0, 0);
+  }
+  double* Uo = Ubuf + U_off;
+#pragma unroll
+  for (int q = 0; q < 4; q++) {
+    double cs = (vok >> q) & 1u ? v[0][q] : 0.0;
+#pragma unroll
+    for (int c = 1; c < MAXC; c++) cs += (vok >> (4 * c + q)) & 1u ? v[c][q] : 0.0;
+    const double acc = -prod[q] + cs;
+    if (!(gi[q] < r && gj <= gi[q])) continue;
+    if (pdst[q]) *pdst[q] = oldv[q] + acc;
+    else Uo[uidx(gi[q], gj, r, my_ra)] = acc;
+  }
+  LTIME_MAX(5);
+}
+
+template <bool BATCH>
+__global__ __launch_bounds__(kFT, 2) void k_front_level_self(const WorkRec* __restrict__ work, int work_begin, int nfactor, int nfactor_pad,
+                                                          const double* __restrict__ PanR, double* __restrict__ Lbuf,
+                                                          double* __restrict__ yvec, double* __restrict__ uvec,
+                                                          int* __restrict__ status, int level_id, int write_l11c, int chunk_rows,
+                                                          const int32_t* __restrict__ tiles_x, int tile_begin, int ntiles,
+                                                          const int32_t* __restrict__ inv, const int32_t* __restrict__ rel,
+                                                          double* __restrict__ Ubuf, double* __restrict__ Pan, long long js) {
+  extern __shared__ __attribute__((aligned(16))) unsigned char smem[];
+  if ((int)blockIdx.x < nfactor_pad) {
+    if ((int)blockIdx.x >= nfactor) return;
+    front_factor_item<BATCH, false>(work, work_begin, PanR, Lbuf, yvec, uvec, status, level_id, write_l11c, chunk_rows, js, nullptr, smem);
+    LTIME_MAX(1);
+    return;
+  }
+  const int t = (int)blockIdx.x - nfactor_pad;
+  if (t >= ntiles) return;
+  front_update_tile_self<kFrontW, BATCH>(work, tiles_x + kSelfTileInts * (size_t)(tile_begin + t), inv, rel, PanR, Ubuf, Pan, js,
+                                         *reinterpret_cast<SelfTileLds<kFrontW>*>(smem), level_id);
+}
+
 __device__ __forceinline__ double4_t mm16(const double* X, int ldx, const double* Y, int ldy, double4_t acc, int lane) {
   const double* xp = X + (lane & 15) * ldx + (lane >> 4);
   const double* yp = Y + (lane >> 4) * ldy + (lane & 15);
@@ -1426,6 +1634,8 @@
       (void)hipFuncSetAttribute(f, hipFuncAttributeMaxDynamicSharedMemorySize, factor_smem_bytes(kChunkRows + 1));
     for (const void* f : {reinterpret_cast<const void*>(k_front_level<false>), reinterpret_cast<const void*>(k_front_level<true>)})
       (void)hipFuncSetAttribute(f, hipFuncAttributeMaxDynamicSharedMemorySize, std::max(factor_smem_bytes(kChunkRows + 1), 2 * (int)sizeof(UpdTileLds<kFrontW>)));
+    for (const void* f : {reinterpret_cast<const void*>(k_front_level_self<false>), reinterpret_cast<const void*>(k_front_level_self<true>)})
+      (void)hipFuncSetAttribute(f, hipFuncAttributeMaxDynamicSharedMemorySize, std::max(factor_smem_bytes(kChunkRows + 1), (int)sizeof(SelfTileLds<kFrontW>)));
 #define CGMR_X(when, ...) reinterpret_cast<const void*>(k_linearize<__VA_ARGS__>),
     for (const void* f : {CGMR_LINEARIZE_TABLE(CGMR_X)})
 #undef CGMR_X
@@ -1459,6 +1669,15 @@
   hipLaunchKernelGGL(CGMR_KERN(D, k_front_level), dim3(nw_pad + ntw, 1, D.njobs), dim3(kFT), level_merge_smem(D, l), st, D.work, D.h_work_ptr[l], nw, nw_pad,
                      D.Pan, D.Lbuf, D.yvec, D.uvec, D.status, l, write_l11c ? 1 : 0, D.h_level_chunk[l], D.tiles, D.h_tile_ptr[l], nt, ntw,
                      D.fronts, D.children, D.inv, D.rel, D.Ubuf, D.Pan, D.ready, spin_limit, D.job_stride);
+}
+void launch_front_level_self(hipStream_t st, const GnDevice& D, int l, bool write_l11c) {
+  gn_init_kernels();
+  const int nw = D.h_work_ptr[l + 1] - D.h_work_ptr[l], nt = D.h_tile_ptr[l + 1] - D.h_tile_ptr[l];
+  const int nw_pad = (nw + 7) / 8 * 8;
+  hipLaunchKernelGGL(CGMR_KERN(D, k_front_level_self), dim3(nw_pad + nt, 1, D.njobs), dim3(kFT),
+                     std::max(factor_smem_bytes(D.h_level_chrows[l]), (int)sizeof(SelfTileLds<kFrontW>)), st, D.work, D.h_work_ptr[l], nw, nw_pad,
+                     D.Pan, D.Lbuf, D.yvec, D.uvec, D.status, l, write_l11c ? 1 : 0, D.h_level_chunk[l], D.tiles_x, D.h_tilex_ptr[l], nt,
+                     D.inv, D.rel, D.Ubuf, D.Pan, D.job_stride);
 }
 int level_merge_wgs(const GnDevice& D, int l) {
   const int nw = D.h_work_ptr[l + 1] - D.h_work_ptr[l], nt = D.h_tile_ptr[l + 1] - D.h_tile_ptr[l];
@@ -1482,8 +1701,13 @@
   int ncu = 0;
   if (hipDeviceGetAttribute(&ncu, hipDeviceAttributeMultiprocessorCount, dev) != hipSuccess) ncu = 0;
   D.h_level_merge.assign(D.nlevels, 0);
+  D.h_level_self.assign(D.nlevels, 0);
   if (!D.sw->fwd_merge || off || kFrontW != 48) return;
   for (int l = 0; l < D.nlevels; l++) {
+    if (level_merge_wgs(D, l) > 0 && l + 1 < (int)D.h_tilex_ptr.size() && D.h_tilex_ptr[l + 1] > D.h_tilex_ptr[l]) D.h_level_self[l] = 1;
+  }
+  for (int l = 0; l < D.nlevels; l++) {
+    if (D.h_level_self[l]) continue;
     const int wgs = level_merge_wgs(D, l), sm = level_merge_smem(D, l);
     const int cls = sm <= 40 * 1024 ? 0 : sm <= 53 * 1024 ? 1 : sm <= 80 * 1024 ? 2 : 3;
     if (wgs > 0 && l < (int)D.h_level_mergeable.size() && D.h_level_mergeable[l] && (any_size || wgs <= per_cu[dev][cls] * ncu / std::max(1, slots_div))) D.h_level_merge[l] = 1;
diff --git a/cg_mrslam_amd/csrc/gn_symbolic.h b/cg_mrslam_amd/csrc/gn_symbolic.h
--- a/cg_mrslam_amd/csrc/gn_symbolic.h
+++ b/cg_mrslam_amd/csrc/gn_symbolic.h
@@ -18,6 +18,8 @@
 
 constexpr int kTopChunkRows = 31;
 constexpr int kTopChunkFronts = 8;
+constexpr int kSelfTileInts = 8;
+constexpr int kFwdSelfTiles = 128;
 constexpr int kLeafChunkRows = 95;
 
 constexpr int kTopMaxCols = 128;
diff --git a/cg_mrslam_amd/csrc/switches.h b/cg_mrslam_amd/csrc/switches.h
--- a/cg_mrslam_amd/csrc/switches.h
+++ b/cg_mrslam_amd/csrc/switches.h
@@ -11,6 +11,7 @@
                                                                                                     \
   X("CGMR_FWD_MERGE", fwd_merge, flag, true, context, "a level's factorisation and update tiles in one launch where it is certainly resident; 0: two launches per level") \
   X("CGMR_FWD_MERGE_ANY", fwd_merge_any, flag, true, context, "merged level launches also where residency is not certain, until the context's first time-out; 0: never") \
+  X("CGMR_FWD_SELF_TILES", fwd_self_tiles, num, kFwdSelfTiles, context, "a merged level above the leaves of at most n update tiles: each tile factors its own rows, nothing waits inside the launch; 0: never") \
   X("CGMR_BWD_CHAIN", bwd_chain, num, -1, context, "at most n workgroups in the chained backward solve; 0: one launch per level; -1: what is certainly resident") \
   X("CGMR_BWD_CHAIN_WGS", bwd_chain_wgs, num, 0, context, "2 / 4: that instance of the chained backward solve (workgroups per CU); else chosen by tree size") \
   X("CGMR_BWD_SPIN_LIMIT", bwd_spin_limit, min1, 1 << 22, context, "polls a bounded device-side wait may take (chained backward solve, merged levels) before it times out") \
diff --git a/include/cgmr.h b/include/cgmr.h
--- a/include/cgmr.h
+++ b/include/cgmr.h
@@ -244,7 +244,7 @@
 
 int cgmr_set_profiling(cgmr_ctx* ctx, int on);
 int cgmr_gn_kernel_times(const cgmr_ctx* ctx, double seconds_out[8], int64_t launches_out[8]);
-int cgmr_gn_kernel_times_ex(const cgmr_ctx* ctx, double seconds_out[12], int64_t launches_out[12]);
+int cgmr_gn_kernel_times_ex(const cgmr_ctx* ctx, double seconds_out[13], int64_t launches_out[13]);
 
 typedef struct cgmr_matcher_config {
   float grid_ll_x, grid_ll_y, grid_ur_x, grid_ur_y;
```

New measurement: 1942 GN iterations/s. -3.1%, worse.
